# WoodwindHu/RangeLDM

Hardware: AMD Instinct MI355X
Metric: range-images/sec, KITTI-360 64x1024 50-step DDIM @ batch16, 1/2/4/8 GPU (higher is better)
Workload: dtype bf16; 1 GPU; RangeLDM (latent 4x256x16), 50-step DDIM + VAE decode (4x), batch 16 per GPU, synthetic weights, x_T resident in HBM; global_batch=16, batch_per_gpu=16, inference_steps=50, sampler=ddim, parallelism=sample-sharded x1, RCCL all-gather of finished images

## Files before the change

### include/rangeldm_hip.h

```cpp
#ifndef RANGELDM_HIP_H
#define RANGELDM_HIP_H

#include <stddef.h>
#include <stdint.h>

#ifdef __cplusplus
extern "C" {
#endif

#define RLDM_MAX_LEVELS 8

typedef struct rldm_unet rldm_unet;
typedef struct rldm_vae rldm_vae;
typedef struct rldm_sampler rldm_sampler;

typedef struct rldm_unet_config {
    int32_t sample_w, sample_h;
    int32_t in_channels, out_channels;
    int32_t layers_per_block;
    int32_t num_levels;
    int32_t block_out_channels[RLDM_MAX_LEVELS];
    int32_t down_attn[RLDM_MAX_LEVELS];
    int32_t up_attn[RLDM_MAX_LEVELS];
    int32_t attention_head_dim;
// ... 257 lines not shown
    const float* cs1;
    const float* gamma;
    const float* beta;
    int32_t silu, groups;
    float eps;
    float* cs_out;
    const float* g0;
    const float* g1;
    int32_t G0;
    const float* gcs0;
    const float* gcs1;
    const float* ggamma;
    const float* gbeta;
    int32_t gsilu, ggroups;
    float geps;
    float* gs_out;
} rldm_train_fuse;
int rldm_train_conv_fused_ok(const rldm_train_conv_desc* d, const rldm_train_fuse* f, int rowadd_ld);
int rldm_train_conv_fused(const rldm_train_conv_desc* d, const rldm_train_fuse* f, const float* x, const void* w_packed,
                          const float* bias, const float* rowadd, int rowadd_ld, const float* res, float* y, int prezeroed,
                          void* stream);
int rldm_train_wgrad_fused_ok(const rldm_train_conv_desc* d, const rldm_train_fuse* f);
int rldm_train_wgrad_fused(const rldm_train_conv_desc* d, const rldm_train_fuse* f, const float* dy, const float* x, float* dw,
                           float* rows, int rows_ld, int rows_accumulate, float* total, void* stream);
int rldm_train_defer_reduce(int on);
int rldm_train_flush_reduce(void);
int rldm_train_reduce_pending(void);
int rldm_train_wgrad_group(int on);
int rldm_train_wgrad_group_flush(void);
int rldm_train_wgrad_group_pending(void);
int rldm_train_deterministic(int on);
int rldm_train_deterministic_enabled(void);
int rldm_train_chan_stats(const float* x, int B, int npix, int C, float* cs, void* stream);
int rldm_train_gn_backward_apply(const float* dz, const float* x0, const float* x1, int C0, const float* cs0, const float* cs1,
                                 const float* gs, int B, int npix, int C, int groups, float eps, const float* gamma,
                                 const float* res, float* dx0, int accumulate0, float* dx1, int accumulate1, float* dgamma,
                                 float* dbeta, void* stream);
int rldm_train_linear_rows(const float* x, int ldx, const void* w_packed, int K, const float* bias, float* y, int ldy, int B, int N,
                           int accumulate, void* stream);
int rldm_train_linear_rows_wgrad(const float* dy, int ldy, const float* x, int ldx, int B, int N, int K, float* dw, float* dbias,
                                 void* stream);
int rldm_train_attention_forward(const float* q, const float* k, const float* v, int B, int L, int C, float* o, float* lse,
                                 void* stream);
int rldm_train_attention_backward(const float* q, const float* k, const float* v, const float* o, const float* dO, const float* lse,
                                  int B, int L, int C, float* delta, float* dq, float* dk, float* dv, void* stream);
int rldm_train_attention_qkv_forward(const float* qkv, int B, int L, int C, float* o, float* lse, void* stream);
int rldm_train_attention_qkv_backward(const float* qkv, const float* o, const float* dO, const float* lse, int B, int L, int C,
                                      float* delta, float* dqkv, void* stream);
int rldm_train_add(const float* a, const float* b, float* y, int64_t n, void* stream);
int rldm_train_copy_channels(const float* src, int src_ld, int src_off, float* dst, int dst_ld, int dst_off, int ncopy,
                             int64_t npix, int accumulate, void* stream);
int rldm_train_sum2x2(const float* du, int B, int W, int H, int C, float* dx, void* stream);
int rldm_train_silu(const float* x, const float* dy, float* y, int64_t n, int backward, int accumulate, void* stream);
int rldm_train_timestep_embedding(const int64_t* timesteps , int B, int dim, float* out, void* stream);
int rldm_train_pack_input(const float* x, int B, int C, int W, int H, int pos_encoding, float* y, void* stream);
int rldm_train_unpack_output(const float* x, int B, int C, int W, int H, float* y, void* stream);
int rldm_train_mse(const float* pred, const float* target, const float* weight, int B, int C, int W, int H, float* dpred,
                   double* loss, void* stream);
int rldm_train_l1(const float* pred, const float* target, const float* wc, int B, int C, int W, int H, float* dpred, double* out,
                  void* stream);
int rldm_train_gaussian(const float* moments, const float* noise, int B, int W, int H, int Z, float* z, double* kl, void* stream);
int rldm_train_gaussian_backward(const float* moments, const float* noise, const float* dz, float kw, int B, int W, int H, int Z,
                                 float* dmoments, void* stream);
int rldm_train_sqnorm(const float* g, int64_t n, double* out , void* stream);
typedef struct rldm_adamw_config {
    float lr, beta1, beta2, eps, weight_decay;
    float max_grad_norm;
    float ema_decay;
    int32_t step;
} rldm_adamw_config;
int rldm_train_adamw(float* params, const float* grads, float* exp_avg, float* exp_avg_sq, float* ema, const double* sqnorm,
                     int64_t n, const rldm_adamw_config* c, void* stream);
int rldm_train_adamw_dyn(float* params, float* grads, float* exp_avg, float* exp_avg_sq, float* ema, const double* sqnorm,
                         int64_t n, const rldm_adamw_config* c, const float* dyn, int zero_grads, void* stream);
typedef struct rldm_hyper_config {
    float lr, beta1, beta2;
    float ema_max_decay, ema_inv_gamma, ema_power;
    int64_t lr_warmup_steps, total_steps;
} rldm_hyper_config;
int rldm_train_hyper_step(int64_t* step_counter, const rldm_hyper_config* c, float* dyn, void* stream);
int rldm_train_pack_weights(const float* w, int N, int Cin, int taps, void* w_forward, void* w_transposed, void* stream);
typedef struct rldm_pack_desc {
    int64_t first;
    int64_t param_offset;
    void* w_forward;
    void* w_transposed;
    int32_t N, Cin, taps, pad_;
} rldm_pack_desc;
int rldm_train_pack_weights_all(const float* params, const rldm_pack_desc* descs, int num_layers, int64_t total, void* stream);
int rldm_train_pack_weights_tiled(const float* params, const rldm_pack_desc* descs, int num_layers, int64_t total_tiles, void* stream);

typedef struct rldm_train_disc_conv_desc {
    int32_t B, Win, Hin, Cin;
    int32_t N;
    int32_t stride;
} rldm_train_disc_conv_desc;
int rldm_train_disc_conv_ok(const rldm_train_disc_conv_desc* d);
int rldm_train_disc_conv(const rldm_train_disc_conv_desc* d, const float* x, const void* w_packed, const float* bias, float* y,
                         void* stream);
int rldm_train_disc_conv_dgrad(const rldm_train_disc_conv_desc* d, const float* dy, const void* w_transposed, float* dx, void* stream);
int64_t rldm_train_disc_wgrad_workspace(const rldm_train_disc_conv_desc* d);
int rldm_train_disc_wgrad(const rldm_train_disc_conv_desc* d, const float* dy, const float* x, float* dw, float* dbias,
                          void* workspace, int64_t workspace_bytes, void* stream);
int64_t rldm_train_disc_bn_workspace(int64_t M, int C);
int rldm_train_disc_bn_forward(const float* x, int64_t M, int C, const float* gamma, const float* beta, float* running_mean,
                               float* running_var, int64_t* num_batches_tracked, int training, float* save, float* y,
                               void* workspace, int64_t workspace_bytes, void* stream);
int rldm_train_disc_bn_backward(const float* x, const float* dy, const float* save, int64_t M, int C, const float* gamma,
                                const float* beta, float* dx, float* dgamma, float* dbeta, void* workspace, int64_t workspace_bytes,
                                void* stream);
int rldm_train_disc_lrelu(const float* x, const float* dy, float* y, int64_t n, int backward, void* stream);
int rldm_train_disc_hinge(const float* real, const float* fake, int64_t n, float factor, float* dreal, float* dfake, double* out,
                          double* partials, void* stream);
int rldm_train_disc_generator(const float* fake, int64_t n, float* dfake, double* out, double* partials, void* stream);
int rldm_train_disc_adaptive_mix(const float* dnll, const float* dg, const double* sq_nll, const double* sq_g, float disc_weight,
                                 float disc_factor, float* dpred, double* d_weight, int64_t n, void* stream);

typedef struct rldm_train_meta_desc {
    int32_t B, Win, Hin, C;
    int32_t N;
    int32_t stride;
} rldm_train_meta_desc;
int rldm_train_meta_ok(const rldm_train_meta_desc* d);
int64_t rldm_train_meta_workspace(const rldm_train_meta_desc* d);
int rldm_train_meta_range(const float* x, int64_t npix, int C, float range_mean, float range_std, float* r, void* stream);
int rldm_train_meta_range_grad(const float* dr, int64_t npix, int C, float range_std, float* dx, void* stream);
int rldm_train_meta_forward(const rldm_train_meta_desc* d, const float* x, const float* r, const float* tables, const float* w1,
                            const float* b1, const float* w2, const float* b2, const float* coov, const float* bias, float* y,
                            float* r_next, float* pe, int32_t* src, float* m, void* workspace, int64_t workspace_bytes, void* stream);
int rldm_train_meta_backward(const rldm_train_meta_desc* d, const float* x, const float* dy, const float* tables, const float* w1,
                             const float* b1, const float* w2, const float* coov, const float* pe, const int32_t* src, const float* m,
                             const float* dr_next, float* dx, float* dr, float* dw1, float* db1, float* dw2, float* db2, float* dcoov,
                             float* dbias, void* workspace, int64_t workspace_bytes, void* stream);

double rldm_unet_flops(rldm_unet* m, int B);
double rldm_vae_decode_flops(rldm_vae* m, int B, int latent_w, int latent_h);
int rldm_unet_num_launches(rldm_unet* m, int B);

int rldm_sampler_profile(rldm_sampler* s, const float* x_T, char* json_out, size_t cap);

typedef struct rldm_conv_desc {
    int32_t B, Cin0, Cin1, Win, Hin;
    int32_t Cout;
    int32_t ksize;
    int32_t stride;
    int32_t pad_mode;
    int32_t upsample;
    int32_t gn;
    int32_t silu;
    float eps;
} rldm_conv_desc;
int rldm_test_conv(const rldm_conv_desc* d, const float* x0, const float* x1, const float* weight, const float* bias,
                   const float* gamma, const float* beta, const float* temb, const float* res, float* y, void* stream);
int rldm_bench_conv(const rldm_conv_desc* d, int with_res, int with_temb, int warmup, int iters, float* avg_us,
                    char* kernel_name, size_t name_cap, void* stream);
int rldm_debug_force_tile(int BM, int BN, int ksplit);
int rldm_unet_trunk_status(rldm_unet* m, int B);
int rldm_unet_set_plan_flags(rldm_unet* m, int flags);
int rldm_debug_inject_trunk_error(rldm_sampler* s, int code);
int rldm_debug_timestamps(unsigned long long* host_out);
int rldm_debug_block_times(unsigned long long* host_out, int nblocks);
enum rldm_flag {
    RLDM_FLAG_ATTN_PROJ_LAUNCH = 1 << 7,
    RLDM_FLAG_NO_CONV_SMALL    = 1 << 8,
    RLDM_FLAG_SMALL_128PX      = 1 << 10,
    RLDM_FLAG_NO_STREAM_REGW   = 1 << 11,
    RLDM_FLAG_STREAM_ANY_GRID  = 1 << 12,
    RLDM_FLAG_GRAPH_TRACE      = 1 << 13,
    RLDM_FLAG_SMALL_64PX_32X2  = 1 << 19,
    RLDM_FLAG_CONSUMER_GN      = 1 << 20,
    RLDM_FLAG_NO_WIDE_SPLIT    = 1 << 21,
    RLDM_FLAG_OWN_IMAGE_COPIES = 1 << 22,
    RLDM_FLAG_SCHED_LAUNCH     = 1 << 23,
    RLDM_FLAG_NO_PERSISTENT    = 1 << 24,
    RLDM_FLAG_NO_CLUSTERS      = 1 << 26
};
int rldm_debug_set_flags(int flags);
enum rldm_flag2 {
    RLDM_FLAG2_STREAM_8WAVE_FULL = 1,
    RLDM_FLAG2_STREAM_8WAVE_128X8 = 2,
    RLDM_FLAG2_STREAM_8WAVE_C64 = 4,
    RLDM_FLAG2_STREAM_SPEC_WAVES = 32,
    RLDM_FLAG2_STREAM_64PX = 64,
    RLDM_FLAG2_NO_REGW = 1 << 24,
    RLDM_FLAG2_REGW_CAP8 = 1 << 25,
    RLDM_FLAG2_FP32_OUT = 1 << 26,
    RLDM_FLAG2_HALO_RING = 1 << 29
};
int rldm_debug_set_flags2(int flags);
int rldm_debug_graph_trace(unsigned long long* stamps, int cap, char* names, size_t names_cap);
int rldm_test_conv_stats(const rldm_conv_desc* d, const float* x0, const float* weight, const float* bias, float* stats,
                         void* stream);
int rldm_test_attention(const float* qkv, int B, int L, int C, float* out, void* stream);
int rldm_test_attention_qkv(const float* x, int B, int L, int C, int groups, float eps, const float* gamma, const float* beta,
                            const float* wqkv, const float* bqkv, float* out, void* stream);
int rldm_test_attention_route(int B, int L, int C, int* route);
int rldm_test_attention_block(const float* x, int B, int L, int C, int groups, float eps, const float* gamma, const float* beta,
                              const float* wqkv, const float* bqkv, const float* to_out_w, const float* to_out_b, int mode, float* y,
                              float* stats, void* stream);
int rldm_bench_attention_qkv(int B, int L, int C, int warmup, int iters, float* avg_us, void* stream);

int rldm_calibrate(double* mfma_tflops, double* mfma_clock_mhz, double* copy_gbs, void* stream);
#define RLDM_CALIB_STAMP_BLOCKS 16
int rldm_calib_clock_stamp(unsigned long long* slots, void* stream);

#ifdef __cplusplus
}
#endif
#endif
```

### rangeldm_amd/_lib.py

```python
import ctypes as C
import enum
import os

_HERE = os.path.dirname(os.path.abspath(__file__))
LIB_PATH = os.environ.get("RLDM_LIB") or os.path.join(_HERE, "librangeldm_hip.so")
RLDM_MAX_LEVELS = 8
RLDM_SAMPLER_DDIM, RLDM_SAMPLER_DDPM, RLDM_SAMPLER_DPMSOLVER = 0, 1, 2
RLDM_EMD_RECT, RLDM_EMD_SYMMETRIC, RLDM_EMD_DIAGONAL = 0, 1, 2
RLDM_EMD_BID_CAP = 2
RLDM_VOXEL_RANGE, RLDM_VOXEL_MAX_SLOTS = 4, 1 << 25
RLDM_HOUGH_MAX_THETA, RLDM_HOUGH_MAX_H, RLDM_HOUGH_MAX_BEAMS = 65536, 4096, 256
RLDM_FRECHET_SWEEP_CAP, RLDM_FRECHET_NONFINITE, RLDM_FRECHET_MAX_SWEEPS = 2, 3, 60
RLDM_FEATURE_MAX_K = 16
RLDM_TRAIN_PAD_END = 4
RLDM_RN_CONV1X1, RLDM_RN_CONV3X3, RLDM_RN_CONV3X3_S2, RLDM_RN_UPCONV = 0, 1, 2, 3


class Flag(enum.IntFlag):
    ATTN_PROJ_LAUNCH = 1 << 7
    NO_CONV_SMALL = 1 << 8
    SMALL_128PX = 1 << 10
    NO_STREAM_REGW = 1 << 11
    STREAM_ANY_GRID = 1 << 12
    GRAPH_TRACE = 1 << 13
    SMALL_64PX_32X2 = 1 << 19
    CONSUMER_GN = 1 << 20
    NO_WIDE_SPLIT = 1 << 21
    OWN_IMAGE_COPIES = 1 << 22
    SCHED_LAUNCH = 1 << 23
    NO_PERSISTENT = 1 << 24
    NO_CLUSTERS = 1 << 26


class Flag2(enum.IntFlag):
    STREAM_8WAVE_FULL = 1
    STREAM_8WAVE_128X8 = 2
    STREAM_8WAVE_C64 = 4
    STREAM_SPEC_WAVES = 32
    STREAM_64PX = 64
    NO_REGW = 1 << 24
    REGW_CAP8 = 1 << 25
    FP32_OUT = 1 << 26
    HALO_RING = 1 << 29


class UNetConfigC(C.Structure):
    _fields_ = [("sample_w", C.c_int32), ("sample_h", C.c_int32), ("in_channels", C.c_int32),
                ("out_channels", C.c_int32), ("layers_per_block", C.c_int32), ("num_levels", C.c_int32),
                ("block_out_channels", C.c_int32 * RLDM_MAX_LEVELS), ("down_attn", C.c_int32 * RLDM_MAX_LEVELS),
                ("up_attn", C.c_int32 * RLDM_MAX_LEVELS), ("attention_head_dim", C.c_int32),
                ("norm_num_groups", C.c_int32), ("norm_eps", C.c_float), ("mid_attention", C.c_int32),
                ("flip_sin_to_cos", C.c_int32), ("freq_shift", C.c_int32)]


class VAEConfigC(C.Structure):
    _fields_ = [("in_channels", C.c_int32), ("out_channels", C.c_int32), ("ch", C.c_int32), ("num_levels", C.c_int32),
                ("ch_mult", C.c_int32 * RLDM_MAX_LEVELS), ("num_res_blocks", C.c_int32), ("z_channels", C.c_int32),
                ("double_z", C.c_int32), ("norm_num_groups", C.c_int32), ("norm_eps", C.c_float),
                ("scaling_factor", C.c_float)]


class SamplerConfigC(C.Structure):
    _fields_ = [("batch", C.c_int32), ("num_steps", C.c_int32), ("mode", C.c_int32), ("pos_encoding", C.c_int32),
                ("cond_channels", C.c_int32), ("guided", C.c_int32), ("coef", C.POINTER(C.c_float)),
                ("timesteps", C.POINTER(C.c_int64)),
                ("plan_flags", C.c_int32), ("prediction_type", C.c_int32)]


class ConvDescC(C.Structure):
    _fields_ = [("B", C.c_int32), ("Cin0", C.c_int32), ("Cin1", C.c_int32), ("Win", C.c_int32), ("Hin", C.c_int32),
                ("Cout", C.c_int32), ("ksize", C.c_int32), ("stride", C.c_int32), ("pad_mode", C.c_int32),
                ("upsample", C.c_int32), ("gn", C.c_int32), ("silu", C.c_int32), ("eps", C.c_float)]


class LidarConfigC(C.Structure):
    _fields_ = [("beams", C.c_int32), ("width", C.c_int32), ("mode", C.c_int32), ("mean", C.c_float), ("std", C.c_float),
                ("range_fill", C.c_float), ("intensity_fill", C.c_float), ("grid", C.c_int32 * 3),
                ("pc_range", C.c_float * 6), ("normalize_volume_densities", C.c_int32)]


class RangeNetLayerDescC(C.Structure):
    _fields_ = [("kind", C.c_int32), ("B", C.c_int32), ("H", C.c_int32), ("W", C.c_int32), ("Cin", C.c_int32),
                ("Cout", C.c_int32), ("leaky", C.c_int32)]


class RangeNetConfigC(C.Structure):
    _fields_ = [("layers", C.c_int32), ("in_channels", C.c_int32), ("num_classes", C.c_int32)]


class TrainConvDescC(C.Structure):
    _fields_ = [("B", C.c_int32), ("Win", C.c_int32), ("Hin", C.c_int32), ("Cin", C.c_int32), ("N", C.c_int32),
                ("taps", C.c_int32), ("stride", C.c_int32), ("mode", C.c_int32)]


class TrainMetaDescC(C.Structure):
    _fields_ = [("B", C.c_int32), ("Win", C.c_int32), ("Hin", C.c_int32), ("C", C.c_int32), ("N", C.c_int32), ("stride", C.c_int32)]


class TrainDiscConvDescC(C.Structure):
    _fields_ = [("B", C.c_int32), ("Win", C.c_int32), ("Hin", C.c_int32), ("Cin", C.c_int32), ("N", C.c_int32), ("stride", C.c_int32)]


class TrainFuseC(C.Structure):
    _fields_ = [("x1", C.c_void_p), ("C0", C.c_int32), ("cs0", C.c_void_p), ("cs1", C.c_void_p), ("gamma", C.c_void_p),
                ("beta", C.c_void_p), ("silu", C.c_int32), ("groups", C.c_int32), ("eps", C.c_float), ("cs_out", C.c_void_p),
                ("g0", C.c_void_p), ("g1", C.c_void_p), ("G0", C.c_int32), ("gcs0", C.c_void_p), ("gcs1", C.c_void_p),
                ("ggamma", C.c_void_p), ("gbeta", C.c_void_p), ("gsilu", C.c_int32), ("ggroups", C.c_int32), ("geps", C.c_float),
                ("gs_out", C.c_void_p)]


class PackDescC(C.Structure):
    _fields_ = [("first", C.c_int64), ("param_offset", C.c_int64), ("w_forward", C.c_void_p), ("w_transposed", C.c_void_p),
                ("N", C.c_int32), ("Cin", C.c_int32), ("taps", C.c_int32), ("pad_", C.c_int32)]


class HyperConfigC(C.Structure):
    _fields_ = [("lr", C.c_float), ("beta1", C.c_float), ("beta2", C.c_float), ("ema_max_decay", C.c_float),
                ("ema_inv_gamma", C.c_float), ("ema_power", C.c_float), ("lr_warmup_steps", C.c_int64), ("total_steps", C.c_int64)]


class AdamWConfigC(C.Structure):
    _fields_ = [("lr", C.c_float), ("beta1", C.c_float), ("beta2", C.c_float), ("eps", C.c_float),
                ("weight_decay", C.c_float), ("max_grad_norm", C.c_float), ("ema_decay", C.c_float), ("step", C.c_int32)]


_P = C.c_void_p
PROTOTYPES = {
    "rldm_last_error": (C.c_char_p, []),
    "rldm_device_info": (C.c_int, [C.c_char_p, C.c_size_t, C.POINTER(C.c_int)]),
    "rldm_unet_create": (C.c_int, [C.POINTER(UNetConfigC), C.POINTER(_P)]),
    "rldm_unet_destroy": (None, [_P]),
    "rldm_unet_set_param": (C.c_int, [_P, C.c_char_p, _P, C.c_int64]),
    "rldm_unet_finalize": (C.c_int, [_P]),
    "rldm_unet_forward": (C.c_int, [_P, _P, _P, C.c_int, C.c_int, _P, _P]),
    "rldm_vae_create": (C.c_int, [C.POINTER(VAEConfigC), C.POINTER(_P)]),
    "rldm_vae_destroy": (None, [_P]),
    "rldm_vae_set_param": (C.c_int, [_P, C.c_char_p, _P, C.c_int64]),
    "rldm_vae_finalize": (C.c_int, [_P]),
    "rldm_vae_decode": (C.c_int, [_P, _P, C.c_int, C.c_int, C.c_int, _P, _P]),
    "rldm_vae_encode": (C.c_int, [_P, _P, C.c_int, C.c_int, C.c_int, _P, _P]),
    "rldm_diag_gaussian_sample": (C.c_int, [_P, _P, C.c_float, C.c_int, C.c_int, C.c_int, _P, _P]),
    "rldm_sched_ddim_step": (C.c_int, [C.POINTER(C.c_float), _P, _P, _P, _P, C.c_int64, _P]),
    "rldm_sched_ddpm_step": (C.c_int, [C.POINTER(C.c_float), _P, _P, _P, _P, C.c_int64, _P]),
    "rldm_sched_step": (C.c_int, [C.c_int, C.c_int, C.POINTER(C.c_float), _P, _P, _P, _P, C.c_int64, _P]),
    "rldm_sched_dpmsolver_step": (C.c_int, [C.c_int, C.POINTER(C.c_float), _P, _P, _P, _P, C.c_int64, _P]),
    "rldm_sched_guided_step": (C.c_int, [C.c_int, C.c_int, C.POINTER(C.c_float), _P, _P, _P, _P, _P, _P, _P, _P, C.c_int, C.c_int,
                                         C.c_int64, _P]),
    "rldm_sched_add_noise": (C.c_int, [_P, _P, C.POINTER(C.c_float), C.POINTER(C.c_float), C.c_int, C.c_int64, _P, _P]),
    "rldm_sampler_create": (C.c_int, [_P, _P, C.POINTER(SamplerConfigC), C.POINTER(_P)]),
    "rldm_sampler_destroy": (None, [_P]),
    "rldm_sample": (C.c_int, [_P, _P, _P, _P, _P, _P, _P]),
    "rldm_sample_guided": (C.c_int, [_P, _P, _P, _P, _P, _P, _P, _P, _P, _P]),
    "rldm_sampler_status": (C.c_int, [_P]),
    "rldm_unet_set_plan_flags": (C.c_int, [_P, C.c_int]),
    "rldm_debug_inject_trunk_error": (C.c_int, [_P, C.c_int]),
    "rldm_comm_bind": (C.c_int, []),
    "rldm_comm_unique_id": (C.c_int, [_P, C.c_size_t]),
    "rldm_comm_create": (C.c_int, [_P, C.c_int, C.c_int, C.POINTER(_P)]),
    "rldm_comm_destroy": (None, [_P]),
    "rldm_comm_info": (C.c_int, [_P, C.POINTER(C.c_int), C.POINTER(C.c_int), C.c_char_p, C.c_size_t]),
    "rldm_allgather_images": (C.c_int, [_P, _P, _P, C.c_int64, _P]),
    "rldm_allreduce_grads": (C.c_int, [_P, _P, C.c_int64, C.c_int, _P]),
    "rldm_lidar_create": (C.c_int, [C.POINTER(LidarConfigC), C.POINTER(C.c_float), C.POINTER(C.c_float), C.POINTER(_P)]),
    "rldm_lidar_destroy": (None, [_P]),
    "rldm_lidar_to_points": (C.c_int, [_P, _P, C.c_int, C.c_int, C.c_int, _P, _P]),
    "rldm_lidar_to_voxel": (C.c_int, [_P, _P, C.c_int, C.c_int, C.c_int, _P, _P]),
    "rldm_lidar_to_voxel_train": (C.c_int, [_P, _P, C.c_int, C.c_int, C.c_int, _P, _P, _P]),
    "rldm_lidar_to_voxel_ordered": (C.c_int, [_P, _P, C.c_int, C.c_int, C.c_int, _P, _P, _P]),
    "rldm_lidar_to_voxel_backward": (C.c_int, [_P, _P, C.c_int, C.c_int, C.c_int, _P, _P, _P, _P, _P]),
    "rldm_lidar_filter_points": (C.c_int, [_P, _P, C.c_int, C.c_int, C.c_int, C.c_float, _P, _P, _P]),
    "rldm_render_u8": (C.c_int, [_P, C.c_int, C.c_int, C.c_int, C.c_int, C.c_int, _P, _P]),
    "rldm_lidar_project": (C.c_int, [_P, _P, C.c_int, C.c_int, _P, C.c_float, _P, _P, _P, _P]),
    "rldm_bev_histogram": (C.c_int, [_P, _P, C.c_int, C.c_int, C.c_float, C.c_int, C.c_float, C.c_float, _P, _P]),
    "rldm_hist_jsd": (C.c_int, [_P, C.c_int, _P, C.c_int, C.c_int, C.POINTER(C.c_double), _P]),
    "rldm_hist_spectral_sq": (C.c_int, [_P, C.c_int, _P, C.c_int, C.c_int, C.c_int, _P, _P]),
    "rldm_hist_mmd": (C.c_int, [_P, C.c_int, _P, C.c_int, C.c_int, C.c_float, C.POINTER(C.c_double), _P]),
    "rldm_chamfer_nn": (C.c_int, [_P, _P, C.c_int, _P, _P, C.c_int, C.c_int, _P, _P, _P]),
    "rldm_chamfer_mean": (C.c_int, [_P, _P, _P, _P, C.c_int, _P, _P, _P]),
    "rldm_nn_index": (C.c_int, [_P, _P, C.c_int, _P, _P, C.c_int, C.c_int, _P, _P, _P, _P, _P, _P, _P]),
    "rldm_knn": (C.c_int, [_P, _P, C.c_int, _P, _P, C.c_int, C.c_int, C.c_int, C.c_int, _P, _P, _P]),
    "rldm_knn_normals": (C.c_int, [_P, _P, C.c_int, C.c_int, _P, C.c_int, _P, _P, _P]),
    "rldm_chamfer_matrix": (C.c_int, [_P, _P, C.c_int, C.c_int, _P, _P, C.c_int, C.c_int, C.c_int, _P, _P, _P]),
    "rldm_matrix_row_argmin": (C.c_int, [_P, C.c_int, C.c_int, C.c_int, _P, _P, _P]),
    "rldm_voxel_counts": (C.c_int, [_P, _P, C.c_int, _P, _P, C.c_int, C.c_int, C.c_float, _P, _P]),
    "rldm_hough_pack": (C.c_int, [_P, C.c_int64, C.c_int, C.c_float, C.c_float, _P, _P]),
    "rldm_hough_vote": (C.c_int, [_P, C.c_int64, _P, C.c_int, C.c_float, C.c_float, C.c_int, _P, _P]),
    "rldm_hough_vote_shape": (C.c_int, [C.c_int64, C.c_int, C.c_int, C.POINTER(C.c_int32), C.POINTER(C.c_int64)]),
    "rldm_hough_row_max": (C.c_int, [_P, C.c_int, C.c_int, _P, _P, _P]),
    "rldm_hough_assign": (C.c_int, [_P, C.c_int64, _P, C.c_int, C.c_float, _P, _P]),
    "rldm_hough_moments": (C.c_int, [_P, _P, C.c_int64, C.c_int, _P, _P, _P]),
    "rldm_emd_matrix": (C.c_int, [_P, _P, C.c_int, C.c_int, _P, _P, C.c_int, C.c_int, C.c_int, C.c_float, _P, _P, _P, _P, _P]),
    "rldm_farthest_point_sample": (C.c_int, [_P, _P, C.c_int, C.c_int, C.c_int, _P, _P, _P]),
    "rldm_gram_f64": (C.c_int, [_P, C.c_int, _P, C.c_int, C.c_int, _P, _P]),
    "rldm_singular_values_f64": (C.c_int, [_P, C.c_int, C.c_int, C.c_double, C.c_int, _P, C.POINTER(C.c_int), _P]),
    "rldm_frechet_distance": (C.c_int, [_P, C.c_int, _P, C.c_int, C.c_int, C.POINTER(C.c_double), _P]),
    "rldm_frechet_last_sweeps": (C.c_int, []),
    "rldm_feature_scan_f64": (C.c_int, [_P, C.c_int, _P, C.c_int, C.c_int, C.c_int, _P, _P, C.c_int, C.c_int, C.c_longlong,
                                        _P, _P, _P, _P, _P, _P]),
    "rldm_feature_scan_column_chunk": (C.c_int, [C.c_int]),
    "rldm_rangenet_packed_elems": (C.c_longlong, [C.c_int, C.c_int, C.c_int]),
    "rldm_rangenet_pack_weights": (C.c_int, [C.c_int, C.c_int, C.c_int, _P, _P]),
    "rldm_rangenet_layer": (C.c_int, [C.POINTER(RangeNetLayerDescC), _P, _P, _P, _P, _P, _P, _P, _P, _P, _P, C.c_int, _P, _P, _P]),
    "rldm_rangenet_num_layers": (C.c_int, [C.POINTER(RangeNetConfigC)]),
    "rldm_rangenet_layer_info": (C.c_int, [C.POINTER(RangeNetConfigC), C.c_int, C.POINTER(RangeNetLayerDescC)]),
    "rldm_rangenet_create": (C.c_int, [C.POINTER(RangeNetConfigC), C.POINTER(_P), C.POINTER(_P), C.POINTER(_P), C.c_int, C.POINTER(_P)]),
    "rldm_rangenet_destroy": (None, [_P]),
    "rldm_rangenet_forward": (C.c_int, [_P, _P, C.c_int, C.c_int, C.c_int, _P, _P, C.c_int, _P, _P, _P, _P]),
    "rldm_rangenet_project": (C.c_int, [_P, _P, C.c_int, C.c_int, C.c_int, C.c_int, C.c_double, C.c_double, C.POINTER(C.c_float),
                                        C.POINTER(C.c_float), _P, _P, _P, _P, _P, _P, _P, _P, _P]),
    "rldm_rangenet_unproject": (C.c_int, [_P, _P, _P, _P, _P, _P, C.c_int, C.c_int, C.c_int, C.c_int, C.c_int, _P, C.c_float,
                                          C.c_int, _P, _P]),
    "rldm_range_errors": (C.c_int, [_P, _P, C.c_int, C.c_int, C.c_int, C.c_int, C.c_int, C.POINTER(C.c_float),
                                    C.POINTER(C.c_float), C.c_int, C.c_int, _P, _P, _P]),
    "rldm_beam_upsample": (C.c_int, [_P, C.c_int, C.c_int, C.c_int, C.c_int, C.c_int, C.c_int, _P, _P]),
    "rldm_train_conv": (C.c_int, [C.POINTER(TrainConvDescC), _P, _P, _P, _P, C.c_int, _P, _P, C.c_int, _P]),
    "rldm_train_conv_splits": (C.c_int, [C.POINTER(TrainConvDescC), C.c_int]),
    "rldm_train_wgrad": (C.c_int, [C.POINTER(TrainConvDescC), _P, _P, _P, _P]),
    "rldm_train_wgrad_bias": (C.c_int, [C.POINTER(TrainConvDescC), _P, _P, _P, _P, C.c_int, C.c_int, _P, _P]),
    "rldm_train_colsum": (C.c_int, [_P, C.c_int, C.c_int, C.c_int, _P, C.c_int, C.c_int, _P, _P]),
    "rldm_train_gn_forward": (C.c_int, [_P, C.c_int, C.c_int, C.c_int, C.c_int, C.c_float, _P, _P, C.c_int, _P, _P, _P]),
    "rldm_train_gn_backward": (C.c_int, [_P, _P, _P, C.c_int, C.c_int, C.c_int, C.c_int, _P, _P, C.c_int, _P, _P, C.c_int,
                                         _P, _P, _P]),
    "rldm_train_conv_fused_ok": (C.c_int, [C.POINTER(TrainConvDescC), C.POINTER(TrainFuseC), C.c_int]),
    "rldm_train_conv_fused": (C.c_int, [C.POINTER(TrainConvDescC), C.POINTER(TrainFuseC), _P, _P, _P, _P, C.c_int, _P, _P, C.c_int, _P]),
    "rldm_train_wgrad_fused_ok": (C.c_int, [C.POINTER(TrainConvDescC), C.POINTER(TrainFuseC)]),
    "rldm_train_wgrad_fused": (C.c_int, [C.POINTER(TrainConvDescC), C.POINTER(TrainFuseC), _P, _P, _P, _P, C.c_int, C.c_int, _P, _P]),
    "rldm_train_defer_reduce": (C.c_int, [C.c_int]),
    "rldm_train_flush_reduce": (C.c_int, []),
    "rldm_calibrate": (C.c_int, [C.POINTER(C.c_double), C.POINTER(C.c_double), C.POINTER(C.c_double), _P]),
    "rldm_calib_clock_stamp": (C.c_int, [_P, _P]),
    "rldm_train_wgrad_group": (C.c_int, [C.c_int]),
    "rldm_train_wgrad_group_flush": (C.c_int, []),
    "rldm_train_wgrad_group_pending": (C.c_int, []),
    "rldm_train_deterministic": (C.c_int, [C.c_int]),
    "rldm_train_deterministic_enabled": (C.c_int, []),
    "rldm_train_reduce_pending": (C.c_int, []),
    "rldm_train_chan_stats": (C.c_int, [_P, C.c_int, C.c_int, C.c_int, _P, _P]),
    "rldm_train_gn_backward_apply": (C.c_int, [_P, _P, _P, C.c_int, _P, _P, _P, C.c_int, C.c_int, C.c_int, C.c_int, C.c_float, _P, _P,
                                               _P, C.c_int, _P, C.c_int, _P, _P, _P]),
    "rldm_train_linear_rows": (C.c_int, [_P, C.c_int, _P, C.c_int, _P, _P, C.c_int, C.c_int, C.c_int, C.c_int, _P]),
    "rldm_train_linear_rows_wgrad": (C.c_int, [_P, C.c_int, _P, C.c_int, C.c_int, C.c_int, C.c_int, _P, _P, _P]),
    "rldm_train_attention_forward": (C.c_int, [_P, _P, _P, C.c_int, C.c_int, C.c_int, _P, _P, _P]),
    "rldm_train_attention_backward": (C.c_int, [_P, _P, _P, _P, _P, _P, C.c_int, C.c_int, C.c_int, _P, _P, _P, _P, _P]),
    "rldm_train_attention_qkv_forward": (C.c_int, [_P, C.c_int, C.c_int, C.c_int, _P, _P, _P]),
    "rldm_train_attention_qkv_backward": (C.c_int, [_P, _P, _P, _P, C.c_int, C.c_int, C.c_int, _P, _P, _P]),
    "rldm_train_add": (C.c_int, [_P, _P, _P, C.c_int64, _P]),
    "rldm_train_copy_channels": (C.c_int, [_P, C.c_int, C.c_int, _P, C.c_int, C.c_int, C.c_int, C.c_int64, C.c_int, _P]),
    "rldm_train_sum2x2": (C.c_int, [_P, C.c_int, C.c_int, C.c_int, C.c_int, _P, _P]),
    "rldm_train_silu": (C.c_int, [_P, _P, _P, C.c_int64, C.c_int, C.c_int, _P]),
    "rldm_train_timestep_embedding": (C.c_int, [_P, C.c_int, C.c_int, _P, _P]),
    "rldm_train_pack_input": (C.c_int, [_P, C.c_int, C.c_int, C.c_int, C.c_int, C.c_int, _P, _P]),
    "rldm_train_unpack_output": (C.c_int, [_P, C.c_int, C.c_int, C.c_int, C.c_int, _P, _P]),
    "rldm_train_mse": (C.c_int, [_P, _P, _P, C.c_int, C.c_int, C.c_int, C.c_int, _P, _P, _P]),
    "rldm_train_l1": (C.c_int, [_P, _P, _P, C.c_int, C.c_int, C.c_int, C.c_int, _P, _P, _P]),
    "rldm_train_gaussian": (C.c_int, [_P, _P, C.c_int, C.c_int, C.c_int, C.c_int, _P, _P, _P]),
    "rldm_train_gaussian_backward": (C.c_int, [_P, _P, _P, C.c_float, C.c_int, C.c_int, C.c_int, C.c_int, _P, _P]),
    "rldm_train_sqnorm": (C.c_int, [_P, C.c_int64, _P, _P]),
    "rldm_train_adamw": (C.c_int, [_P, _P, _P, _P, _P, _P, C.c_int64, C.POINTER(AdamWConfigC), _P]),
    "rldm_train_adamw_dyn": (C.c_int, [_P, _P, _P, _P, _P, _P, C.c_int64, C.POINTER(AdamWConfigC), _P, C.c_int, _P]),
    "rldm_train_hyper_step": (C.c_int, [_P, C.POINTER(HyperConfigC), _P, _P]),
    "rldm_train_pack_weights": (C.c_int, [_P, C.c_int, C.c_int, C.c_int, _P, _P, _P]),
    "rldm_train_pack_weights_all": (C.c_int, [_P, _P, C.c_int, C.c_int64, _P]),
    "rldm_train_pack_weights_tiled": (C.c_int, [_P, _P, C.c_int, C.c_int64, _P]),
    "rldm_train_disc_conv_ok": (C.c_int, [C.POINTER(TrainDiscConvDescC)]),
    "rldm_train_disc_conv": (C.c_int, [C.POINTER(TrainDiscConvDescC), _P, _P, _P, _P, _P]),
    "rldm_train_disc_conv_dgrad": (C.c_int, [C.POINTER(TrainDiscConvDescC), _P, _P, _P, _P]),
    "rldm_train_disc_wgrad_workspace": (C.c_int64, [C.POINTER(TrainDiscConvDescC)]),
    "rldm_train_disc_wgrad": (C.c_int, [C.POINTER(TrainDiscConvDescC), _P, _P, _P, _P, _P, C.c_int64, _P]),
    "rldm_train_disc_bn_workspace": (C.c_int64, [C.c_int64, C.c_int]),
    "rldm_train_disc_bn_forward": (C.c_int, [_P, C.c_int64, C.c_int, _P, _P, _P, _P, _P, C.c_int, _P, _P, _P, C.c_int64, _P]),
    "rldm_train_disc_bn_backward": (C.c_int, [_P, _P, _P, C.c_int64, C.c_int, _P, _P, _P, _P, _P, _P, C.c_int64, _P]),
    "rldm_train_disc_lrelu": (C.c_int, [_P, _P, _P, C.c_int64, C.c_int, _P]),
    "rldm_train_disc_hinge": (C.c_int, [_P, _P, C.c_int64, C.c_float, _P, _P, _P, _P, _P]),
    "rldm_train_disc_generator": (C.c_int, [_P, C.c_int64, _P, _P, _P, _P]),
    "rldm_train_disc_adaptive_mix": (C.c_int, [_P, _P, _P, _P, C.c_float, C.c_float, _P, _P, C.c_int64, _P]),
    "rldm_train_meta_ok": (C.c_int, [C.POINTER(TrainMetaDescC)]),
    "rldm_train_meta_workspace": (C.c_int64, [C.POINTER(TrainMetaDescC)]),
    "rldm_train_meta_range": (C.c_int, [_P, C.c_int64, C.c_int, C.c_float, C.c_float, _P, _P]),
    "rldm_train_meta_range_grad": (C.c_int, [_P, C.c_int64, C.c_int, C.c_float, _P, _P]),
    "rldm_train_meta_forward": (C.c_int, [C.POINTER(TrainMetaDescC)] + [_P] * 15 + [C.c_int64, _P]),
    "rldm_train_meta_backward": (C.c_int, [C.POINTER(TrainMetaDescC)] + [_P] * 20 + [C.c_int64, _P]),
    "rldm_unet_flops": (C.c_double, [_P, C.c_int]),
    "rldm_vae_decode_flops": (C.c_double, [_P, C.c_int, C.c_int, C.c_int]),
    "rldm_unet_num_launches": (C.c_int, [_P, C.c_int]),
    "rldm_unet_trunk_status": (C.c_int, [_P, C.c_int]),
    "rldm_sampler_profile": (C.c_int, [_P, _P, C.c_char_p, C.c_size_t]),
    "rldm_test_conv": (C.c_int, [C.POINTER(ConvDescC), _P, _P, _P, _P, _P, _P, _P, _P, _P, _P]),
    "rldm_bench_conv": (C.c_int, [C.POINTER(ConvDescC), C.c_int, C.c_int, C.c_int, C.c_int, C.POINTER(C.c_float),
                                  C.c_char_p, C.c_size_t, _P]),
    "rldm_debug_force_tile": (C.c_int, [C.c_int, C.c_int, C.c_int]),
    "rldm_test_conv_stats": (C.c_int, [C.POINTER(ConvDescC), _P, _P, _P, _P, _P]),
    "rldm_debug_set_flags": (C.c_int, [C.c_int]),
    "rldm_debug_set_flags2": (C.c_int, [C.c_int]),
    "rldm_debug_graph_trace": (C.c_int, [_P, C.c_int, C.c_char_p, C.c_size_t]),
    "rldm_debug_timestamps": (C.c_int, [_P]),
    "rldm_debug_block_times": (C.c_int, [_P, C.c_int]),
    "rldm_test_attention": (C.c_int, [_P, C.c_int, C.c_int, C.c_int, _P, _P]),
    "rldm_test_attention_qkv": (C.c_int, [_P, C.c_int, C.c_int, C.c_int, C.c_int, C.c_float, _P, _P, _P, _P, _P, _P]),
    "rldm_test_attention_route": (C.c_int, [C.c_int, C.c_int, C.c_int, C.POINTER(C.c_int)]),
    "rldm_test_attention_block": (C.c_int, [_P, C.c_int, C.c_int, C.c_int, C.c_int, C.c_float, _P, _P, _P, _P, _P, _P, C.c_int, _P, _P,
                                            _P]),
    "rldm_bench_attention_qkv": (C.c_int, [C.c_int, C.c_int, C.c_int, C.c_int, C.c_int, C.POINTER(C.c_float), _P]),
}

_lib = None


def lib():
    global _lib
    if _lib is None:
        if not os.path.exists(LIB_PATH):
            raise RuntimeError(f"{LIB_PATH} not found: build it with `python -c 'import __graft_entry__ as g; g.build()'` "
                               f"(hipcc --offload-arch=gfx950).  rangeldm_amd has no CPU fallback.")
        import torch
        L = C.CDLL(LIB_PATH)
        for name, (res, args) in PROTOTYPES.items():
            fn = getattr(L, name)
            fn.restype = res
            fn.argtypes = args
        _lib = L
    return _lib


def check(rc, what=""):
    if rc != 0:
        msg = lib().rldm_last_error()
        raise RuntimeError(f"librangeldm_hip: {what} failed: {msg.decode() if msg else 'unknown error'}")


def stream_ptr(device=None):
    import torch
    return C.c_void_p(torch.cuda.current_stream(device).cuda_stream)


def require_gpu():
    import torch
    if not torch.cuda.is_available():
        raise RuntimeError("rangeldm_amd needs an MI355X (gfx950) visible to PyTorch-ROCm; there is no CPU fallback")
    name = C.create_string_buffer(64)
    cus = C.c_int(0)
    check(lib().rldm_device_info(name, 64, C.byref(cus)), "rldm_device_info")
    return name.value.decode(), cus.value
```

### rangeldm_amd/csrc/conv_stream.hip

```cpp
#include "conv_stream_body.h"
#include "conv_stream_spec_body.h"

#include <utility>

namespace rldm {

template <int WM, int WN, int NW, int MI, int S, bool SUB, bool T4, bool FH>
__global__ void __launch_bounds__((StreamInstDesc{WM, WN, NW, MI}.threads()), (StreamInstDesc{WM, WN, NW, MI}.wg_per_cu())) conv_stream_kernel(const ConvParams p) {
    int nt, mt, b;
    {
        const int gx = p.ntile_n, gy = p.tiles_img;
        const int lin = blockIdx.x + gx * (blockIdx.y + gy * blockIdx.z);
        const int rid = (p.dbg & (1 << 21)) ? lin : xcd_remap(lin, gx * gy * p.B);
        const int q = rid / gx;
        nt = rid - q * gx;
        b = q / gy;
        mt = q - b * gy;
    }
    const TrunkSeam none = {};
    conv_stream_body<WM, WN, false, NW, MI, S, SUB, T4, FH>(p, nt, mt, b, none);
}

__global__ void __launch_bounds__(512, 1) conv_stream_spec_kernel(const ConvParams p) {
    int nt, mt, b;
    {
        const int gx = p.ntile_n, gy = p.tiles_img;
        const int lin = blockIdx.x + gx * (blockIdx.y + gy * blockIdx.z);
        const int rid = (p.dbg & (1 << 21)) ? lin : xcd_remap(lin, gx * gy * p.B);
        const int q = rid / gx;
        nt = rid - q * gx;
        b = q / gy;
        mt = q - b * gy;
    }
    const TrunkSeam none = {};
    conv_stream_spec_body<false>(p, nt, mt, b, none);
}

int conv_stream_bn(const ConvParams& p) { return stream_inst(p).bn(); }
int conv_stream_kgroups(const ConvParams& p) { return stream_inst(p).kgroups(); }
int conv_stream_threads(const ConvParams& p) { return stream_inst(p).threads(); }

size_t conv_stream_lds_bytes(const ConvParams& p) {
    const int BN = conv_stream_bn(p), KG = conv_stream_kgroups(p), BM = p.TW * p.TH;
    const size_t a = (size_t)((p.TW - 1) * p.stride + 3) * p.colb;
    const size_t main_bytes = 2 * a + (size_t)(p.C0 + p.C1) * 8 + BN * 4;
    const size_t gscratch = p.st0 ? (size_t)2 * (p.C0 + p.C1) * 8 : 0;
    const size_t epi = KG == 1 ? (size_t)BM * (BN * 2 + 16) + (size_t)8 * 2 * BN * 4
                               : (size_t)KG * 64 * (BN * 4 + 16) + (size_t)64 * (BN * 2 + 16) + (size_t)8 * 2 * BN * 4;
    return std::max(std::max(main_bytes, gscratch), epi);
}

bool conv_stream_supported(const ConvParams& p, int taps) {
    if (p.st_inst < 0 || p.st_inst >= SI_COUNT) return false;
    const StreamInstDesc& d = stream_inst(p);
    const int Cin = p.C0 + p.C1, R = p.R0 + p.R1;
    if (taps != 9 || p.pad_lo != 1 || (p.up != 1 && p.up != 2) || p.y_nchw || p.ksplit > 1) return false;
    if (Cin % 64 != 0 || (p.C1 != 0 && p.C0 % 64 != 0) || R % 64 != 0 || (p.R1 != 0 && p.R0 % 64 != 0)) return false;
    if (R != 0 && p.up != 1) return false;
    if (p.Win * p.up < 2 || p.N % d.bn() != 0 || Cin > 512) return false;
    if (p.st0 && (p.gn_groups > 64 || Cin % p.gn_groups != 0)) return false;
    if ((p.tiles_h & (p.tiles_h - 1)) != 0 || p.B > 65535 || p.tiles_img > 65535) return false;
    if (p.stride != d.STR || !d.takes(p.TW, p.TH) || (d.up1 && p.up != 1) || (d.no_res && R != 0)) return false;
    if (d.SUB && (p.Wout != 2 * p.Win || p.Hout != 2 * p.Hin)) return false;
    if (d.FH && p.Hout != p.TH) return false;
    return conv_stream_lds_bytes(p) <= (size_t)d.lds_cap();
}

template <int I>
static int launch_stream_inst(const ConvParams& p, size_t lds, hipStream_t stream) {
    constexpr StreamInstDesc d = kStreamInst[I];
    void (*kern)(const ConvParams);
    if constexpr (d.spec) kern = conv_stream_spec_kernel;
    else kern = conv_stream_kernel<d.WM, d.WN, d.NW, d.MI, d.STR, d.SUB, d.T4, d.FH>;
    static DynLdsLimit lds_limit;
    RLDM_HIP_CHECK(lds_limit.ensure(reinterpret_cast<const void*>(kern), lds));
    hipLaunchKernelGGL(kern, dim3(p.N / d.bn() * (d.SUB ? 4 : 1), p.tiles_img, p.B), dim3(d.threads()), lds, stream, p);
    RLDM_HIP_CHECK(hipGetLastError());
    return 0;
}
template <int... I>
static int launch_stream_row(const ConvParams& p, size_t lds, hipStream_t stream, std::integer_sequence<int, I...>) {
    static constexpr int (*launch[])(const ConvParams&, size_t, hipStream_t) = {launch_stream_inst<I>...};
    return launch[p.st_inst](p, lds, stream);
}

int launch_conv_stream(const ConvParams& p, hipStream_t stream) {
    RLDM_REQUIRE(conv_stream_supported(p, 9), "conv_stream: unsupported shape");
    return launch_stream_row(p, conv_stream_lds_bytes(p), stream, std::make_integer_sequence<int, SI_COUNT>());
}

}
```

### rangeldm_amd/csrc/kernels.h

```cpp
#pragma once
#include "common.h"

namespace rldm {

struct NormView {
    bf16_t* y;
    const float* gamma;
    const float* beta;
    int ld;
    int cpg_shift;
    float inv_n;
    float eps;
    int silu;
};

constexpr int kSchedMultistep = 8;
__device__ __forceinline__ float sched_prev(const int mode, const float c0, const float c1, const float c2, const float c3, const float x,
                                            const float e, float& x0_out) {
    const int pred = (mode >> 1) & 3;
    float x0, pe;
    if (pred == 0) {
        x0 = (x - c1 * e) / c0;
        pe = e;
    } else if (pred == 1) {
        x0 = c0 * x - c1 * e;
        pe = c0 * e + c1 * x;
    } else {
        x0 = e;
        pe = (x - c0 * e) / c1;
    }
    x0_out = x0;
    return (mode & 1) == 0 ? c2 * x0 + c3 * pe : c2 * x0 + c3 * x;
}
__device__ __forceinline__ float* sched_history(const int mode, const float* slot) {
    return (mode & kSchedMultistep) ? const_cast<float*>(slot) : nullptr;
}

struct SchedFuse {
    const float* coef_table;
    const int* step_ptr;
    const float* x;
    const float* noise;
    long long noise_step_stride;
    float* x_prev;
    int mode;
    bf16_t* pack;
    int pack_ld;
};

struct ConvParams {
    const bf16_t* x0;
    const bf16_t* x1;
    int C0, C1;
    const bf16_t* r0;
    const bf16_t* r1;
    int R0, R1;
    int B, Win, Hin;
    int up;
    int stride;
    int pad_lo;
    int Wout, Hout;
    int TW, TH;
    int colb;
    int tiles_h, tiles_img;
    int th_shift;
    int magic_thv;
    int magic_cpg;
    const float2* st0;
    const float2* st1;
    int P0, P1;
    int gn_groups;
    const float* gn_gamma;
    const float* gn_beta;
    float gn_eps;
    int silu;
    const bf16_t* wpk;
    int N;
    int ntile_n;
    const float* bias;
    const float* temb;
    int temb_ld;
    const int* step_ptr;
    int temb_rows_per_step;
    int temb_per_sample;
    bf16_t* y;
    int y_ld;
    float2* y_stats;
    float* y_nchw;
    int ksplit;
    float* slab;
    int* ticket;
    int lds_total;
    float gn_inv_n;
    const bf16_t* res;
    unsigned long long* ts;
    int dbg;
    SchedFuse sch;
    int* step_inc;
    int nviews;
    NormView nv[3];
    int st_inst;
    int exp;
    int* cu_lock;
};

struct ConvTile {
    int BM, BN, CK, taps;
};
inline int conv_row_bytes(int CK) { return CK * 2 + 16; }
size_t conv_lds_bytes(const ConvTile& t, const ConvParams& p);
bool conv_tile_supported(const ConvTile& t);
int conv_max_halo_slots(const ConvTile& t);
int conv_halo_col_bytes(const ConvTile& t, int TH, int stride);
int conv_tile_threads(const ConvTile& t);
int launch_conv(const ConvTile& t, const ConvParams& p, hipStream_t stream);

int conv_small_kgroups(int BN);
int conv_small_col_bytes(int Cin, int TH, int taps);
size_t conv_small_lds_bytes(const ConvParams& p, int taps, int BN);
bool conv_small_supported(const ConvParams& p, int taps, int BN);
int launch_conv_small(const ConvParams& p, int taps, int BN, hipStream_t stream);

enum StreamInst : int {
    SI_256x128,
    SI_256x64,
    SI_128x64,
    SI_256x128_SPEC,
    SI_64x128,
    SI_64x128_S2,
    SI_128x128_W4,
    SI_128x64_W4,
    SI_SUB_W4,
    SI_SUB_T4_W4,
    SI_FULLH_W4,
    SI_COUNT
};
enum TrunkStreamForm : int { TSF_NONE = -1, TSF_PLAIN = 0, TSF_SUB = 1, TSF_FULLH = 2 };
struct StreamTile {
    int TW, TH;
};
struct StreamInstDesc {
    int WM, WN, NW = 8, MI = 4, STR = 1;
    bool SUB = false, T4 = false, FH = false;
    bool spec = false;
    StreamTile tiles[2] = {};
    bool up1 = false, no_res = false;
    int trunk = TSF_NONE;
    constexpr int threads() const { return 64 * NW; }
    constexpr int kgroups() const { return NW / (WM * WN); }
    constexpr int bm() const { return 32 * MI * WM; }
    constexpr int bn() const { return 32 * WN; }
    constexpr int wg_per_cu() const { return NW == 4 ? 2 : 1; }
    constexpr int lds_cap() const { return 160 * 1024 / wg_per_cu(); }
    constexpr bool takes(int TW, int TH) const { return (tiles[0].TW == TW && tiles[0].TH == TH) || (tiles[1].TW == TW && tiles[1].TH == TH); }
};
constexpr StreamInstDesc kStreamInst[SI_COUNT] = {
     {2, 4, 8, 4, 1, false, false, false, false, {{32, 8}},          false, false, TSF_PLAIN},
     {2, 2, 8, 4, 1, false, false, false, false, {{32, 8}}},
     {1, 2, 8, 4, 1, false, false, false, false, {{16, 8}, {32, 4}}},
     {2, 4, 8, 4, 1, false, false, false, true,  {{32, 8}}},
     {1, 4, 8, 2, 1, false, false, false, false, {{8, 8}}},
     {1, 4, 8, 2, 2, false, false, false, false, {{8, 8}, {16, 4}},  true,  true},
     {1, 4, 4, 4, 1, false, false, false, false, {{16, 8}},          false, false, TSF_PLAIN},
     {1, 2, 4, 4, 1, false, false, false, false, {{16, 8}}},
     {1, 4, 4, 4, 1, true,  false, false, false, {{16, 8}},          true,  true,  TSF_SUB},
     {1, 4, 4, 4, 1, true,  true,  false, false, {{32, 4}},          true,  true},
     {1, 4, 4, 4, 1, false, false, true,  false, {{8, 16}, {16, 8}}, true,  false, TSF_FULLH},
};
inline const StreamInstDesc& stream_inst(const ConvParams& p) { return kStreamInst[p.st_inst]; }
int conv_stream_bn(const ConvParams& p);
int conv_stream_kgroups(const ConvParams& p);
size_t conv_stream_lds_bytes(const ConvParams& p);
bool conv_stream_supported(const ConvParams& p, int taps);
int launch_conv_stream(const ConvParams& p, hipStream_t stream);

size_t conv_regw_lds_bytes();
int conv_regw_wg_per_image(const ConvParams& p);
int conv_regw_partials(const ConvParams& p);
bool conv_regw_supported(const ConvParams& p);
int launch_conv_regw(const ConvParams& p, hipStream_t stream);
size_t conv_c16_lds_bytes();
bool conv_c16_supported(const ConvParams& p);
int launch_conv_c16(const ConvParams& p, hipStream_t stream);
size_t conv_o4_lds_bytes();
bool conv_o4_supported(const ConvParams& p);
int launch_conv_o4(const ConvParams& p, hipStream_t stream);
size_t conv_ds2_lds_bytes();
bool conv_ds2_supported(const ConvParams& p);
int launch_conv_ds2(const ConvParams& p, hipStream_t stream);

struct TrunkPhase;
struct TrunkParams {
    const TrunkPhase* phases;
    int nphases;
    int B, ranks;
    int ntile_n, nwn;
    int variant;
    int skew;
    unsigned* counters;
    int* error;
    const float* temb;
    const int* step_ptr;
    int temb_rows_per_step, temb_per_sample, temb_ld;
    unsigned long long* ts;
};
int launch_trunk(const TrunkParams& tp, size_t lds, hipStream_t stream);
int trunk_max_resident(int variant, size_t lds);

struct GnStatsParams {
    const bf16_t* x;
    int C;
    int B, npix;
    int P;
    float2* part;
};
int launch_gn_stats(const GnStatsParams& p, hipStream_t stream);

struct GnFoldParams {
    const float2* part;
    float2* out;
    int B, P, C;
};
int launch_gn_fold(const GnFoldParams& p, hipStream_t stream);

struct GnApplyParams {
    const bf16_t* x0;
    const bf16_t* x1;
    int C0, C1;
    const float2* st0;
    const float2* st1;
    int P0, P1;
    int B, npix;
    int groups;
    const float* gamma;
    const float* beta;
    float eps;
    int silu;
    bf16_t* y;
    float inv_n;
    bf16_t* y1;
    int ysplit;
};
int launch_gn_apply(const GnApplyParams& p, hipStream_t stream);

struct AttnParams {
    const bf16_t* qkv;
    bf16_t* out;
    int B, L, C;
};
int launch_attention(const AttnParams& p, hipStream_t stream);

struct AttnQkvParams {
    const bf16_t* x;
    const float2* st;
    int P;
    const float* gamma;
    const float* beta;
    float eps;
    int groups;
    float inv_n;
    int magic_cpg;
    const bf16_t* wfrag;
    const float* bias;
    bf16_t* out;
    int B, L, C;
    unsigned long long* ts;
    int ts_L;
    const bf16_t* proj_w;
    const float* proj_bias;
    const bf16_t* proj_res;
    bf16_t* proj_y;
    float2* proj_stats;
    unsigned* proj_counter;
    int* proj_error;
};
int launch_attention_qkv(const AttnQkvParams& p, hipStream_t stream);
int attention_qkv2_geometry(int B, int L, int C, int* HG, int* waves);
bool attention_proj_fusable(int B, int L, int C, int cus);
int launch_attention_proj(const AttnQkvParams& p, hipStream_t stream);
void attention_qkv_route(int B, int L, int C, int cus, int* route);
constexpr int kAttnXRowBytes = 128 + 16, kAttnXStageBytes = 32 * kAttnXRowBytes;
inline size_t attention_qkv2_lds_bytes(int L, int C, int HG, int waves) {
    const size_t Lp = (size_t)(L + 31) / 32 * 32;
    const size_t a = (size_t)2 * C * 8, b2 = (size_t)HG * (C / 16) * 64 * 4;
    return HG * Lp * 16 + (size_t)HG * 10 * (Lp + 8) * 2 + 16 + (size_t)C * 8 + (a > b2 ? a : b2) + (size_t)HG * C * 64 +
           (size_t)HG * 128 + (size_t)waves * kAttnXStageBytes + 128;
}

struct PackInputParams {
    const float* x; int cx; float scale;
    int pos_encoding;
    const float* cond; int cc;
    int B, W, H, Cpad;
    bf16_t* out;
    int* step_inc;
};
int launch_pack_input(const PackInputParams& p, hipStream_t stream);
int launch_nchw_f32_to_nhwc_bf16(const float* src, bf16_t* dst, int B, int C, int W, int H, int Cpad, hipStream_t s);
int launch_nhwc_bf16_to_nchw_f32(const bf16_t* src, float* dst, int B, int C, int W, int H, int ld, hipStream_t s);

struct TembParams {
    const float* t;
    int rows, dim0, D, total;
    const float* w1; const float* b1;
    const float* w2; const float* b2;
    const float* wp; const float* bp;
    float* out;
    float* scratch;
    int flip_sin_to_cos, freq_shift;
};
int launch_temb(const TembParams& p, hipStream_t stream);

struct SchedParams {
    int mode;
    float coef[5];
    const float* coef_table;
    const int* step_ptr;
    const float* eps; const float* x; const float* noise;
    long long noise_step_stride;
    float* x_prev;
    long long n;
};
int launch_sched_step(const SchedParams& p, hipStream_t stream);
struct GuidedSchedParams {
    SchedParams s;
    float k[4];
// ... 19 lines not shown
```

### rangeldm_amd/csrc/runtime.hip

```cpp
#include "../../include/rangeldm_hip.h"
#include "kernels.h"
#include "trunk_seam.h"

#include <algorithm>
#include <atomic>
#include <cmath>
#include <cstdlib>
#include <cstring>
#include <functional>
#include <map>
#include <memory>
#include <mutex>
#include <tuple>
#include <vector>

namespace rldm {

static thread_local std::string g_error;
void set_error(const std::string& msg) { g_error = msg; }

struct DevBuf {
    void* p = nullptr;
    size_t bytes = 0;
    DevBuf() = default;
// ... 127 lines not shown
            RLDM_REQUIRE(ksize == 3 && (Cout % 32 == 0 || Cout < 32) && Cin_pad % 64 == 0 && R % 64 == 0, "conv " + name + ": not stream-packable");
            const int SPT = 4 / KG, NCC = Cin_pad / 64, NCB = R / 64, nsteps = (NCC * 9 + NCB) * SPT;
            const int ntile32 = (Cout + 31) / 32;
            img.assign((size_t)ntile32 * KG * nsteps * 512 + 16384, 0);
            auto at = [&](int n, int ks, int step, int k) -> bf16_t& {
                const size_t stream = (size_t)(n / 32) * KG + ks / SPT;
                return img[((stream * nsteps + step + ks % SPT) * 64 + (k / 8) * 32 + n % 32) * 8 + k % 8];
            };
            for (int n = 0; n < Cout; ++n) {
                for (int c = 0; c < Cin; ++c)
                    for (int tap = 0; tap < 9; ++tap) at(n, (c % 64) / 16, ((c / 64) * 9 + tap) * SPT, c % 16) = f32_to_bf16(weight(n, c, tap));
                for (int c = 0; c < R; ++c) at(n, (c % 64) / 16, (NCC * 9 + c / 64) * SPT, c % 16) = f32_to_bf16(res_weight(n, c));
            }
            bias.resize((size_t)ntile32 * 32, 0.f);
            return 0;
        });
    }

    int get_c16packed(Packed** out) {
        return cached({WeightLayout::C16, 0, 0}, 16, out, [&](std::vector<bf16_t>& img, std::vector<float>&) {
            RLDM_REQUIRE(ksize == 3 && Cout % 32 == 0 && Cin <= 16 && R == 0, "conv " + name + ": not a 16-channel input layer");
            img.assign((size_t)(Cout / 32) * 9 * 512, 0);
            for (int n = 0; n < Cout; ++n)
                for (int c = 0; c < Cin; ++c)
                    for (int tap = 0; tap < 9; ++tap)
                        img[(((size_t)(n / 32) * 9 + tap) * 64 + (c / 8) * 32 + n % 32) * 8 + c % 8] = f32_to_bf16(weight(n, c, tap));
            return 0;
        });
    }

    int get_subpixpacked(int Cin_pad, Packed** out) {
        return cached({WeightLayout::SubPixel, 0, 0}, Cin_pad, out, [&](std::vector<bf16_t>& img, std::vector<float>&) {
            RLDM_REQUIRE(ksize == 3 && Cout % 32 == 0 && Cin_pad % 64 == 0 && R == 0, "conv " + name + ": not sub-pixel-packable");
            const int NCC = Cin_pad / 64, nsteps = NCC * 16;
            img.assign((size_t)(Cout / 32) * 4 * nsteps * 512 + 16384, 0);
            static const int lo[2][2] = {{0, 1}, {0, 2}}, hi[2][2] = {{0, 2}, {1, 2}};
            for (int n = 0; n < Cout; ++n)
                for (int c = 0; c < Cin; ++c)
                    for (int pw = 0; pw < 2; ++pw)
                        for (int ph = 0; ph < 2; ++ph)
                            for (int i = 0; i < 2; ++i)
                                for (int j = 0; j < 2; ++j) {
                                    float v = 0.f;
                                    for (int a = lo[pw][i]; a <= hi[pw][i]; ++a)
                                        for (int bb = lo[ph][j]; bb <= hi[ph][j]; ++bb) v += weight(n, c, a * 3 + bb);
                                    const size_t stream = (size_t)(n / 32) * 4 + pw * 2 + ph;
                                    const int step = ((c / 64) * 4 + i * 2 + j) * 4 + (c % 64) / 16, k = c % 16;
                                    img[((stream * nsteps + step) * 64 + (k / 8) * 32 + n % 32) * 8 + k % 8] = f32_to_bf16(v);
                                }
            return 0;
        });
    }

    int get_fragpacked(int Cin_pad, int TN, int KG, bool no_res, Packed** out) {
        const WeightLayout layout = no_res ? WeightLayout::FragNoRes : WeightLayout::Frag;
        return cached({layout, TN, KG}, Cin_pad, out, [&](std::vector<bf16_t>& img, std::vector<float>&) {
            const int taps = ksize * ksize, Rp = no_res ? 0 : R, KS = 512 / TN;
            RLDM_REQUIRE((TN == 32 || TN == 16) && Cout % TN == 0 && Cin_pad % (KS * KG) == 0 && Rp % (KS * KG) == 0,
                         "conv " + name + ": not fragment-packable");
            const int CPT = Cin_pad / KS / KG, RPT = Rp / KS / KG, nmine = taps * CPT + RPT;
            img.assign((size_t)(Cout / TN) * KG * nmine * 512 + 512, 0);
            auto at = [&](int n, int step0, int c) -> bf16_t& {
                const int cg = c / KS, k = c % KS;
                const size_t stream = (size_t)(n / TN) * KG + cg % KG;
                return img[((stream * nmine + step0 + cg / KG) * 64 + (k / 8) * TN + n % TN) * 8 + k % 8];
            };
            for (int n = 0; n < Cout; ++n) {
                for (int c = 0; c < Cin; ++c)
                    for (int tap = 0; tap < taps; ++tap) at(n, tap * CPT, c) = f32_to_bf16(weight(n, c, tap));
                for (int c = 0; c < Rp; ++c) at(n, taps * CPT, c) = f32_to_bf16(res_weight(n, c));
            }
            return 0;
        });
    }
};

struct ParamStore {
    std::map<std::string, std::vector<float>> host;
    std::map<std::string, int64_t> expected;
    bool finalized = false;

    int set(const char* name, const float* data, int64_t numel) {
        auto it = expected.find(name);
        RLDM_REQUIRE(it != expected.end(), std::string("unexpected parameter key: ") + name);
        RLDM_REQUIRE(it->second == numel, std::string("size mismatch for ") + name + ": expected " +
                                              std::to_string(it->second) + " got " + std::to_string(numel));
        host[name].assign(data, data + numel);
        finalized = false;
        return 0;
    }
    int check_complete() const {
        for (auto& kv : expected)
            RLDM_REQUIRE(host.count(kv.first), std::string("missing parameter key: ") + kv.first);
        return 0;
    }
    void expect_conv(const std::string& n, int co, int ci, int k) {
        expected[n + ".weight"] = (int64_t)co * ci * k * k;
        expected[n + ".bias"] = co;
    }
    void expect_lin(const std::string& n, int co, int ci) {
        expected[n + ".weight"] = (int64_t)co * ci;
        expected[n + ".bias"] = co;
    }
    void expect_norm(const std::string& n, int c) {
        expected[n + ".weight"] = c;
        expected[n + ".bias"] = c;
    }
    void expect_resnet(const std::string& p, int ci, int co, int temb) {
        expect_norm(p + ".norm1", ci);
        expect_conv(p + ".conv1", co, ci, 3);
        if (temb) expect_lin(p + ".time_emb_proj", co, temb);
        expect_norm(p + ".norm2", co);
        expect_conv(p + ".conv2", co, co, 3);
        if (ci != co) expect_conv(p + ".conv_shortcut", co, ci, 1);
    }
    void expect_attn(const std::string& p, int c) {
        expect_norm(p + ".group_norm", c);
        expect_lin(p + ".to_q", c, c);
        expect_lin(p + ".to_k", c, c);
        expect_lin(p + ".to_v", c, c);
        expect_lin(p + ".to_out.0", c, c);
    }
};

struct Tensor {
    size_t off = 0;
    int B = 0, W = 0, H = 0, C = 0;
    int id = -1;
    size_t st_off = 0;
    int P = 0;
    int prod = -1;
    size_t st_bytes() const { return (size_t)B * P * C * sizeof(float2); }
    size_t bytes() const { return (size_t)B * W * H * C * sizeof(bf16_t); }
    bool valid() const { return id >= 0; }
};

struct PlanIO {
    const float* sample = nullptr;
    int sample_channels = 0;
    float sample_scale = 1.f;
    int pos_encoding = 0;
    const float* cond = nullptr;
    int cond_channels = 0;
    float* out = nullptr;
    const float* temb = nullptr;
    const int* step_ptr = nullptr;
    int temb_rows_per_step = 1;
    int temb_per_sample = 0;
    int* step_inc = nullptr;
    SchedFuse sch = {};
    bool pack_fused = false;
    bf16_t* xin = nullptr;
    int xin_ld = 0;
};

struct Op {
    std::function<int(hipStream_t)> fn;
    std::string name;
    double flops = 0;
    double bytes = 0;
    std::function<bool()> active;
    std::string tag;
};

struct KernelStat {
    int launches = 0;
    double ms = 0, flops = 0, bytes = 0;
};

struct Plan {
    int B = 0, W = 0, H = 0;
    int flags = 0;
    DevBuf arena;
    DevBuf tickets;
    std::vector<std::unique_ptr<DevBuf>> trunk_bufs;
    DevBuf trunk_error;
    PlanIO io;
    std::vector<Op> ops;
    double flops = 0;
    int run(hipStream_t s) {
        for (auto& o : ops)
            if ((!o.active || o.active()) && o.fn(s)) return 1;
        return 0;
    }
    int run_stamped(hipStream_t s, unsigned long long* slots, int cap) {
        if (launch_stamp(slots, s)) return 1;
        int n = 0;
        for (size_t i = 0; i < ops.size(); ++i) {
            if (ops[i].active && !ops[i].active()) continue;
            if (ops[i].fn(s)) return 1;
            ++n;
            if (n < cap && launch_stamp(slots + n, s)) return 1;
        }
        return 0;
    }
    int run_profiled(hipStream_t s, std::map<std::string, KernelStat>& stats) {
        std::vector<hipEvent_t> ev(ops.size() + 1);
        for (auto& e : ev) RLDM_HIP_CHECK(hipEventCreate(&e));
        RLDM_HIP_CHECK(hipEventRecord(ev[0], s));
        std::vector<char> ran(ops.size(), 1);
        for (size_t i = 0; i < ops.size(); ++i) {
            ran[i] = !ops[i].active || ops[i].active();
            if (ran[i] && ops[i].fn(s)) return 1;
            RLDM_HIP_CHECK(hipEventRecord(ev[i + 1], s));
        }
        RLDM_HIP_CHECK(hipStreamSynchronize(s));
        for (size_t i = 0; i < ops.size(); ++i) {
            if (!ran[i]) continue;
            float ms = 0.f;
            RLDM_HIP_CHECK(hipEventElapsedTime(&ms, ev[i], ev[i + 1]));
            KernelStat& k = stats[ops[i].name];
            k.launches += 1;
            k.ms += ms;
            k.flops += ops[i].flops;
            k.bytes += ops[i].bytes;
        }
        for (auto& e : ev) (void)hipEventDestroy(e);
        return 0;
    }
};

struct Layers {
    std::map<std::string, std::unique_ptr<ConvLayer>> conv;
    std::map<std::string, std::unique_ptr<NormParams>> norm;
    ConvLayer* get_conv(const std::string& n) {
        auto it = conv.find(n);
        return it == conv.end() ? nullptr : it->second.get();
    }
    NormParams* get_norm(const std::string& n) {
        auto it = norm.find(n);
        return it == norm.end() ? nullptr : it->second.get();
    }
    int add_conv(ParamStore& ps, const std::string& n, int co, int ci, int k) {
        auto L = std::make_unique<ConvLayer>();
        L->name = n;
        L->Cout = co;
        L->Cin = ci;
        L->ksize = k;
        L->w = ps.host.at(n + ".weight");
        L->b = ps.host.at(n + ".bias");
        conv[n] = std::move(L);
        return 0;
    }
    int add_norm(ParamStore& ps, const std::string& n, int c) {
        auto N = std::make_unique<NormParams>();
        N->C = c;
        if (upload(N->gamma, ps.host.at(n + ".weight").data(), c * sizeof(float))) return 1;
        if (upload(N->beta, ps.host.at(n + ".bias").data(), c * sizeof(float))) return 1;
        norm[n] = std::move(N);
        return 0;
    }
    int add_qkv(ParamStore& ps, const std::string& p, int c, int head_dim) {
        auto L = std::make_unique<ConvLayer>();
        L->name = p + ".qkv";
        L->Cout = 3 * c;
        L->Cin = c;
        L->ksize = 1;
        const float qs = 1.4426950408889634f / std::sqrt((float)head_dim);
        const char* names[3] = {".to_q", ".to_k", ".to_v"};
        for (int i = 0; i < 3; ++i) {
            const auto& w = ps.host.at(p + names[i] + ".weight");
            const auto& b = ps.host.at(p + names[i] + ".bias");
            const float s = i == 0 ? qs : 1.f;
            for (float v : w) L->w.push_back(v * s);
            for (float v : b) L->b.push_back(v * s);
        }
        conv[L->name] = std::move(L);
        return 0;
    }
};

static void pack_attn_head_frags(const float* w, const float* b, int C, std::vector<bf16_t>& img, std::vector<float>& bias) {
    const int heads = C / 8, nks = C / 16;
    img.assign((size_t)heads * nks * 512, 0);
    bias.assign((size_t)heads * 32, 0.f);
    for (int h = 0; h < heads; ++h)
        for (int row = 0; row < 24; ++row) {
            const int src = (row / 8) * C + h * 8 + row % 8;
            bias[(size_t)h * 32 + row] = b[src];
            for (int c = 0; c < C; ++c)
                img[(((size_t)h * nks + c / 16) * 64 + ((c % 16) / 8) * 32 + row) * 8 + c % 8] = f32_to_bf16(w[(size_t)src * C + c]);
        }
}

struct ConvArgs {
    ConvLayer* layer = nullptr;
    Tensor x0, x1;
    int stride = 1, pad_mode = 0, up = 1;
    NormParams* gn = nullptr;
    float eps = 1e-5f;
    int groups = 32;
    int silu = 0;
    int temb_off = -1;
    Tensor r0, r1;
    bool want_stats = false;
    bool out_f32_nchw = false;
    bool own_image = false;
    bool first_of_step = false;
};

struct ConvShape {
    int Cin_t, R_t, taps, Wout, Hout;
};
static ConvShape conv_shape(const ConvArgs& a) {
    return {a.x0.C + (a.x1.valid() ? a.x1.C : 0), (a.r0.valid() ? a.r0.C : 0) + (a.r1.valid() ? a.r1.C : 0),
            a.layer->ksize * a.layer->ksize, a.x0.W * a.up / a.stride, a.x0.H * a.up / a.stride};
}
static double conv_flops(const ConvArgs& a, const ConvShape& s) {
    const ConvLayer* L = a.layer;
    return 2.0 * (double)a.x0.B * s.Wout * s.Hout * L->Cout * ((double)L->Cin * s.taps + (L->sc_identity ? 0.0 : (double)L->R));
}
static double conv_bytes(const ConvArgs& a, const ConvShape& s, size_t out_copies = 1, bool res_weights = true) {
    const ConvLayer* L = a.layer;
    const double out_px = (double)a.x0.B * s.Wout * s.Hout;
    return (double)a.x0.B * a.x0.W * a.x0.H * s.Cin_t * 2.0 + (double)L->Cout * (L->Cin * s.taps + (res_weights ? L->R : 0)) * 2.0 +
           out_px * L->Cout * (a.out_f32_nchw ? 4.0 : 2.0) * (double)out_copies + out_px * s.R_t * 2.0;
}

struct ConvLate {
    int temb_off = -1;
    bool first_of_step = false;
    bool f32_out = false;
    bool sch = false;
    void apply(ConvParams& p, const PlanIO& io) const {
        if (first_of_step) p.step_inc = io.pack_fused ? io.step_inc : nullptr;
        if (temb_off >= 0) {
            p.temb = io.temb + temb_off;
            p.step_ptr = io.step_ptr;
            p.temb_rows_per_step = io.temb_rows_per_step;
            p.temb_per_sample = io.temb_per_sample;
        }
        if (f32_out) p.y_nchw = io.out;
        if (sch) p.sch = io.sch;
    }
};

struct ViewPlan {
    struct Part { int prod; int ch_off; };
    struct Cons {
        std::vector<Part> parts;
        int Ctot = 0, silu = 0, groups = 32;
        float eps = 1e-5f;
        bool ok = false;
        bool use = false;
    };
    struct Emit { const NormParams* norm; int ch_off; int Ctot; int silu; int groups; float eps; };
    std::vector<char> can_emit;
    std::vector<int> out_c;
    std::map<const NormParams*, Cons> cons;
    std::map<int, std::vector<Emit>> emit;
    void decide() {
        std::map<int, int> nper;
        for (auto& kv : cons) {
            Cons& c = kv.second;
            bool good = c.ok && c.groups > 0 && c.Ctot % c.groups == 0;
            const int cpg = good ? c.Ctot / c.groups : 0;
            good = good && cpg >= 1 && cpg <= 32 && (cpg & (cpg - 1)) == 0;
            for (auto& pt : c.parts)
                good = good && pt.prod >= 0 && pt.prod < (int)can_emit.size() && can_emit[pt.prod] && pt.ch_off % cpg == 0 &&
                       nper[pt.prod] < 3;
            c.use = good;
            if (!good) continue;
            for (auto& pt : c.parts) {
                emit[pt.prod].push_back({kv.first, pt.ch_off, c.Ctot, c.silu, c.groups, c.eps});
                nper[pt.prod]++;
            }
        }
    }
};

static int g_dbg_flags = getenv("RLDM_DBG_FLAGS") ? atoi(getenv("RLDM_DBG_FLAGS")) : 0;
static thread_local int t_plan_flags = 0;
static inline int dbg() { return g_dbg_flags | t_plan_flags; }
static int g_dbg_flags2 = 0;
static inline int dbg2() { return g_dbg_flags2; }
static inline int kernel_dbg() {
#ifdef RLDM_ABLATE
    return dbg();
#else
    return 0;
#endif
}
static unsigned long long* g_ts_buf = nullptr;
struct StampEnv {
    const char *trunk, *trunk_first, *attn_l, *ord;
};
static const StampEnv& stamp_env() {
    static const StampEnv e = {getenv("RLDM_TS_TRUNK"), getenv("RLDM_TS_TRUNK_FIRST"), getenv("RLDM_TS_ATTN_L"), getenv("RLDM_TS_ORD")};
    return e;
}
enum class StampSite { Conv, Attn, TestAttn, Trunk };
static unsigned long long* stamp_buf(StampSite site, int n = 0) {
    const StampEnv& e = stamp_env();
    switch (site) {
        case StampSite::Conv:     return e.ord ? (atoi(e.ord) == n ? g_ts_buf : nullptr) : (e.attn_l || e.trunk) ? nullptr : g_ts_buf;
        case StampSite::Attn:     return (e.trunk || e.ord) ? nullptr : g_ts_buf;
        case StampSite::TestAttn: return e.trunk ? nullptr : g_ts_buf;
        case StampSite::Trunk:    return (e.trunk && atoi(e.trunk) == n) ? g_ts_buf : nullptr;
    }
    return nullptr;
}
static constexpr int kInst4MinBlocks = 96;
static int g_force_bm = 0, g_force_bn = 0, g_force_ks = 0;
static constexpr int kGraphSteps = 10;

static thread_local int g_concurrent_plans = 1;

struct TileChoice {
    ConvTile tile;
    int TW = 1, TH = 1, ksplit = 1;
};

static void pixel_tile(int BM, int Wout, int Hout, int* TW, int* TH) {
    int th = 1;
    while (th * 2 <= Hout && th * 2 <= 16 && Hout % (th * 2) == 0) th *= 2;
    int tw = 1;
    while (tw * 2 * th <= BM && Wout % (tw * 2) == 0) tw *= 2;
    *TW = tw;
    *TH = th;
}

static TileChoice choose_tile(long long B, int Wout, int Hout, int stride, int N, int Cin_pad, int C0, int R, int R0,
                              int taps, bool nchw, bool gn) {
    TileChoice c;
    const int KW = taps == 9 ? 3 : 1;
    auto ck_ok = [&](int ck) { return Cin_pad % ck == 0 && C0 % ck == 0 && R % ck == 0 && R0 % ck == 0; };
    auto pick = [&](int BM, int BN, ConvTile* u, int* tw, int* th) {
        const int cks[3] = {64, 32, 16};
        for (int ck : cks) {
            if (!ck_ok(ck)) continue;
            ConvTile v;
            v.BM = BM; v.BN = BN; v.CK = ck; v.taps = taps;
            if (!conv_tile_supported(v)) continue;
            pixel_tile(BM, Wout, Hout, tw, th);
            bool ok = true;
            while (((*tw - 1) * stride + KW) * ((*th - 1) * stride + KW) > conv_max_halo_slots(v)) {
                if (*tw > 1) *tw >>= 1; else if (*th > 1) *th >>= 1; else { ok = false; break; }
            }
            if (!ok) continue;
            *u = v;
            return true;
        }
        return false;
    };
    auto blocks = [&](const ConvTile& u, int tw, int th) {
        return B * (Wout / tw) * (Hout / th) * ((N + u.BN - 1) / u.BN);
    };
    const int bn_pref = N <= 32 ? 32 : (N <= 64 ? 64 : 128);
    const int bms[3] = {256, 128, 64};
    std::vector<int> bns = {bn_pref};
    if (bn_pref > 64) bns.push_back(64);
    long long best_blocks = -1;
    TileChoice best;
    bool found = false;
    for (int pass = 0; pass < 3 && best_blocks < 0; ++pass) {
        if (pass == 2) bns = {32, 64, 128};
        for (int bi = 0; bi < 3 && !found; ++bi)
            for (size_t ni = 0; ni < bns.size() && !found; ++ni) {
                ConvTile u;
                int tw, th;
                if (!pick(bms[bi], bns[ni], &u, &tw, &th)) continue;
                if (pass == 0 && tw * th * 2 <= u.BM && bi < 2 && !(stride == 2 && bi == 0)) continue;
                const long long nb = blocks(u, tw, th);
                if (nb > best_blocks) {
                    best_blocks = nb;
                    best.tile = u;
                    best.TW = tw;
                    best.TH = th;
                }
                if (nb >= ((taps == 1 && gn) ? 128 : 200)) found = true;
            }
    }
    if (g_force_bm && g_force_bn) {
        ConvTile u;
        int tw, th;
        if (pick(g_force_bm, g_force_bn, &u, &tw, &th)) {
            best.tile = u;
            best.TW = tw;
            best.TH = th;
            best_blocks = blocks(u, tw, th);
        }
    }
    c = best;
    if (best_blocks < 0) {
        c.tile.BM = 64; c.tile.BN = 64; c.tile.CK = 16; c.tile.taps = taps;
        return c;
    }
    c.ksplit = 1;
    const int ncc = Cin_pad / c.tile.CK;
    if (!nchw && g_force_ks > 0 && g_force_ks <= std::max(1, ncc)) c.ksplit = g_force_ks;
    return c;
}

struct Builder {
    Plan* plan;
    bool dry;
    Arena arena;
    int next_id = 0;
    std::map<int, int> refs;
    std::map<int, Tensor> live;
    char* base = nullptr;
    int launches = 0;
    int temb_ld = 0;
    int* ticket_ptr = nullptr;
    int tickets = 0;
    ViewPlan* vp = nullptr;
    bool recording = false;
    int conv_ord = 0;
    int groups_hint = 32;
    std::map<const NormParams*, Tensor> view_tensors;
    const std::vector<ViewPlan::Emit>* cur_emit = nullptr;

    void record_consumer(const NormParams* n, const Tensor& x0, const Tensor& x1, int silu, bool ok, int groups, float eps) {
        if (!vp || !recording || !n) return;
        ViewPlan::Cons c;
        c.parts.push_back({x0.prod, 0});
        if (x1.valid()) c.parts.push_back({x1.prod, x0.C});
        c.Ctot = x0.C + (x1.valid() ? x1.C : 0);
        c.silu = silu;
        c.groups = groups;
        c.eps = eps;
        c.ok = ok && x0.W * x0.H == (x1.valid() ? x1.W * x1.H : x0.W * x0.H);
        vp->cons[n] = c;
    }
    bool take_view(const NormParams* n, Tensor* v) {
        if (!vp || recording || !n) return false;
        auto it = vp->cons.find(n);
        if (it == vp->cons.end() || !it->second.use) return false;
// ... 362 lines not shown
                           (taps == 1 && Cin_t == 256) ? TK_CL_1x1_256 : -1;
        const int ranks_c = cluster_ranks(x0.B, N, Wout * Hout);
        const bool in_cluster = !in_trunk && cluster_enabled() && !a.own_image && kind_c >= 0 && BN == 64 && px_t == 64 &&
                                (p.up == 1 || p.up == 2) && vts.empty() && ranks_c == (N / 64) * p.tiles_img &&
                                p.Win * p.up == Wout && p.Hin * p.up == Hout;
        if (preact) {
            const bool gn_phase = gn_phase_t || (in_cluster && Cin_t <= 512 && (Wout * Hout) % ranks_c == 0 && a.x0.C % 8 == 0 &&
                                                 (!a.x1.valid() || a.x1.C % 8 == 0));
            if (gn_phase_t) trunk_begin(x0.B, ranks_t);
            else if (gn_phase) trunk_begin(x0.B, ranks_c, N / 64, 2);
            else note_launch();
            if (!dry) {
                GnApplyParams g;
                memset(&g, 0, sizeof(g));
                g.x0 = tptr(a.x0); g.x1 = tptr(a.x1);
                g.C0 = a.x0.C; g.C1 = a.x1.valid() ? a.x1.C : 0;
                g.st0 = sptr(a.x0); g.st1 = sptr(a.x1);
                g.P0 = a.x0.P; g.P1 = a.x1.valid() ? a.x1.P : 0;
                g.B = a.x0.B; g.npix = a.x0.W * a.x0.H;
                g.groups = a.groups;
                g.gamma = a.gn->gamma.as<float>(); g.beta = a.gn->beta.as<float>();
                g.eps = a.eps; g.silu = a.silu;
                g.y = tptr(act);
                const double by = (double)g.B * g.npix * Cin_t * 4.0;
                if (gn_phase) {
                    g.inv_n = (float)(1.0 / ((double)g.npix * (Cin_t / g.groups)));
                    pend.phases.push_back(trunk_gn_apply_phase(g));
                    pend.lds = std::max(pend.lds, (size_t)(2 * 512 * 8 + 2 * 512 * 4));
                    pend.bytes += by;
                }
                emit({[g](hipStream_t st) { return launch_gn_apply(g, st); }, "gn_apply_kernel", 0.0, by}, gn_phase);
            }
        }
        if (in_trunk) trunk_begin(x0.B, ranks_t);
        else if (in_cluster) trunk_begin(x0.B, ranks_c, N / 64, 2);
        else note_launch();
        in_trunk = in_trunk || in_cluster;
        if (!dry) {
            ConvLayer::Packed* pk = nullptr;
            if (L->get_fragpacked(Cin_t, BN == 16 ? 16 : 32, BN == 16 ? 8 : conv_small_kgroups(BN), epi_res, &pk)) return 1;
            ConvArgs k = a;
            k.x0 = x0;
            if (!gn_fused) k.gn = nullptr;
            if (!gn_fused || p.C1 == 0) k.x1 = Tensor();
            if (epi_res) {
                p.res = tptr(a.r0);
                k.r0 = k.r1 = Tensor();
            }
            bind_conv(p, k, *pk, y);
            for (size_t v = 0; v < vts.size(); ++v) {
                const auto& e = (*cur_emit)[v];
                NormView& nv = p.nv[v];
                nv.y = tptr(vts[v]) + e.ch_off;
                nv.gamma = e.norm->gamma.as<float>() + e.ch_off;
                nv.beta = e.norm->beta.as<float>() + e.ch_off;
                nv.ld = e.Ctot;
                const int cpg = e.Ctot / e.groups;
                nv.cpg_shift = 0;
                while ((1 << nv.cpg_shift) < cpg) ++nv.cpg_shift;
                nv.inv_n = (float)(1.0 / ((double)Wout * Hout * cpg));
                nv.eps = e.eps;
                nv.silu = e.silu;
            }
            p.nviews = (int)vts.size();
            Plan* pl = plan;
            const int temb_off = a.temb_off;
            const double by = conv_bytes(a, s, 1 + vts.size());
            const std::string kname = "conv_small_kernel<" + std::to_string(p.TW * p.TH) + "," + std::to_string(BN) + ",taps" + std::to_string(taps) + ">";
            if (in_trunk) {
                RLDM_REQUIRE(!in_cluster || p.nviews == 0, "conv " + L->name + ": a multi-tile cluster phase writes no views");
                TrunkPhase ph = trunk_conv_phase(p, in_cluster ? kind_c : trunk_kind, in_cluster, temb_off);
                const int KG = in_cluster ? 4 : 8, ksc = BN == 16 ? 32 : 16, cpt = Cin_t / (ksc * KG);
                int G;
                if (in_cluster) G = (taps == 1 ? 1 : (cpt <= 2 ? 9 : (cpt <= 4 ? 3 : 1))) * cpt;
                else G = BN == 16 ? (taps == 9 ? 9 : 1) * cpt : ((trunk_kind & 3) == 0 ? 18 : ((trunk_kind & 3) == 1 ? 12 : cpt));
                ph.w[TW_G] = std::min(G, kTrunkPrefetch);
                ph.w[TW_NMINE] = taps * cpt + ((p.R0 + p.R1) / ksc) / KG;
                ph.w[TW_WBYTES] = (unsigned)((N / (in_cluster ? 32 : BN)) * KG * ph.w[TW_NMINE]) * 1024u;
                pend.phases.push_back(ph);
                pend.lds = std::max(pend.lds, conv_small_lds_bytes(p, taps, BN));
                pend.flops += fl;
                pend.bytes += by;
            }
            const ConvLate late{temb_off};
            emit({[p, BN, taps, pl, late](hipStream_t st) mutable {
                late.apply(p, pl->io);
                return launch_conv_small(p, taps, BN, st);
            }, kname, fl, by}, in_trunk);
        }
        if (preact) release(act);
        *out = y;
        return 0;
    }

    static constexpr int kSubMinBlocks = 96;
    static constexpr long long kAnyGrid = 1ll << 40;
    static bool stream_params_tw(const ConvArgs& a, const ConvShape& s, StreamInst inst, long long min_blocks, long long max_blocks,
                                 ConvParams* q, StreamTile tile = {}) {
        const StreamInstDesc& d = kStreamInst[inst];
        if (tile.TW == 0) tile = d.tiles[0];
        const int TW = tile.TW, TH = tile.TH;
        if (dbg() & RLDM_FLAG_NO_STREAM_REGW) return false;
        if (s.taps != 9 || a.stride != d.STR || a.pad_mode != 0 || a.out_f32_nchw || g_force_bm) return false;
        const bool sub = d.SUB;
        ConvShape tiled = s;
        if (sub) {
            if (a.up != 2 || s.R_t != 0 || s.Wout != 2 * a.x0.W || s.Hout != 2 * a.x0.H) return false;
            tiled.Wout = a.x0.W; tiled.Hout = a.x0.H;
        }
        if (tiled.Wout % TW != 0 || tiled.Hout % TH != 0) return false;
        conv_geometry(a, tiled, TW, TH, d.FH ? TH : (TH - 1) * a.stride + 3, q);
        if (sub) {
            q->up = 1;
            q->Wout = s.Wout; q->Hout = s.Hout;
        }
        q->st_inst = inst;
        ConvTile t;
        t.BM = 256; t.BN = 128; t.CK = 64; t.taps = 9;
        q->colb = conv_halo_col_bytes(t, TH, a.stride);
        const long long blocks = (long long)q->B * q->tiles_img * (q->N / d.bn()) * (sub ? 4 : 1);
        return supported_with(*q, a.gn != nullptr, false, [](const ConvParams& c) { return conv_stream_supported(c, 9); }) &&
               ((dbg() & RLDM_FLAG_STREAM_ANY_GRID) || (blocks >= min_blocks && blocks <= max_blocks));
    }
    static bool stream_params(const ConvArgs& a, const ConvShape& s, ConvParams* q) {
        const int R_t = s.R_t, Hout = s.Hout;
        const auto fits = [&](StreamInst inst, long long min_blocks, long long max_blocks, StreamTile tile = {}) {
            return stream_params_tw(a, s, inst, min_blocks, max_blocks, q, tile);
        };
        const int N_ = a.layer->Cout;
        const bool n128 = N_ % 128 == 0;
        if (a.stride == 2) {
            if (!n128 || R_t != 0 || a.up != 1) return false;
            if (fits(SI_64x128_S2, kInst4MinBlocks, 512, {8, 8})) return true;
            return Hout == 4 && fits(SI_64x128_S2, 48, 512, {16, 4});
        }
        const int f2 = dbg2();
        const StreamInst px256 = n128 ? SI_256x128 : SI_256x64;
        if ((f2 & RLDM_FLAG2_STREAM_SPEC_WAVES) && n128 && fits(SI_256x128_SPEC, 200, kAnyGrid)) return true;
        if ((f2 & RLDM_FLAG2_STREAM_64PX) && n128 && fits(SI_64x128, 192, 512)) return true;
        if (!(f2 & RLDM_FLAG2_STREAM_8WAVE_FULL) && a.up == 2 && n128 &&
            (fits(SI_SUB_W4, kSubMinBlocks, kAnyGrid) || (a.x0.H % 8 != 0 && fits(SI_SUB_T4_W4, kSubMinBlocks, kAnyGrid)))) return true;
        if (!(f2 & (RLDM_FLAG2_STREAM_8WAVE_FULL | RLDM_FLAG2_HALO_RING)) && n128 && (Hout == 16 || Hout == 8) && a.up == 1 &&
            fits(SI_FULLH_W4, 384, kAnyGrid, {Hout == 16 ? 8 : 16, Hout})) return true;
        if (!(f2 & RLDM_FLAG2_STREAM_8WAVE_FULL) && n128 && fits(SI_128x128_W4, 384, kAnyGrid)) return true;
        if (!(f2 & RLDM_FLAG2_STREAM_8WAVE_C64) && !n128 && fits(SI_128x64_W4, 384, kAnyGrid)) return true;
        if (fits(px256, 200, kAnyGrid)) return true;
        if (n128 && Hout == 8 && fits(SI_64x128, kInst4MinBlocks, 320)) return true;
        if (!(f2 & RLDM_FLAG2_STREAM_8WAVE_128X8) && fits(SI_128x64_W4, 257, 512)) return true;
        if (fits(SI_128x64, 128, 512, {16, 8})) return true;
        if (Hout % 8 != 0 && fits(SI_128x64, 128, 512, {32, 4})) return true;
        return fits(px256, 128, kAnyGrid);
    }

    int conv_stream(const ConvArgs& a, const ConvShape& s, ConvParams p, Tensor* out) {
        ConvLayer* L = a.layer;
        const int N = L->Cout;
        const Tensor& x0 = a.x0;
        if (require_gn_input(a, s.Cin_t)) return 1;
        p.dbg = kernel_dbg();
        p.ts = stamp_buf(StampSite::Conv, conv_ord - 1);
        const StreamInstDesc& d = stream_inst(p);
        const bool sub = d.SUB;
        p.ntile_n = N / d.bn() * (sub ? 4 : 1);
        Tensor y = make(x0.B, s.Wout, s.Hout, N);
        if (a.want_stats) add_stats(y, p.tiles_img * (sub ? 4 : 1));
        const double fl_ref = conv_flops(a, s);
        plan->flops += fl_ref;
        const double fl = sub ? fl_ref * 4.0 / 9.0 : fl_ref;
        const int ranks_s = p.tiles_img * p.ntile_n;
        const int per_cu = d.wg_per_cu();
        const bool in_stream_cluster = cluster_enabled() && ranks_s >= 2 && ranks_s <= 16 * per_cu &&
                                       trunk_grid_fits(ranks_s, x0.B, per_cu) && y.P <= kFoldAboveP && N % 128 == 0 &&
                                       d.trunk != TSF_NONE && (!sub || N == 128) && conv_stream_lds_bytes(p) <= (size_t)d.lds_cap();
        if (in_stream_cluster) trunk_begin(x0.B, ranks_s, sub ? 1 : p.ntile_n, 4, d.NW == 4 ? 4 : 2);
        else note_launch();
        if (!dry) {
            ConvLayer::Packed* pk = nullptr;
            if (sub ? L->get_subpixpacked(s.Cin_t, &pk) : L->get_streampacked(s.Cin_t, d.kgroups(), &pk)) return 1;
            bind_conv(p, a, *pk, y);
            Plan* pl = plan;
            const int temb_off = a.temb_off;
            const double by = conv_bytes(a, s);
            if (in_stream_cluster) {
                pend.phases.push_back(trunk_conv_phase(p, TK_STREAM, true, temb_off));
                pend.lds = std::max(pend.lds, conv_stream_lds_bytes(p));
                pend.flops += fl;
                pend.bytes += by;
            }
            const ConvLate late{temb_off};
            emit({[p, pl, late](hipStream_t st) mutable {
                late.apply(p, pl->io);
                return launch_conv_stream(p, st);
            }, "conv_stream_kernel<" + std::to_string(p.TW * p.TH) + "," + std::to_string(d.bn()) + ",CK64,taps9" + (p.stride == 2 ? ",s2" : "") + (sub ? ",sub" : "") + ">", fl, by}, in_stream_cluster);
        }
        *out = y;
        return 0;
    }

    static bool c16_params(const ConvArgs& a, const ConvShape& s, ConvParams* q) {
        const int Cin_t = s.Cin_t, R_t = s.R_t, taps = s.taps, Wout = s.Wout, Hout = s.Hout;
        if ((dbg() & RLDM_FLAG_NO_STREAM_REGW) || g_force_bm || taps != 9 || a.stride != 1 || a.pad_mode != 0 || a.up != 1 || a.out_f32_nchw) return false;
        if (a.x1.valid() || a.gn || a.temb_off >= 0 || R_t != 0 || Cin_t != 16 || a.layer->Cout % 128 != 0 || Wout % 16 != 0 || Hout % 8 != 0) return false;
        conv_geometry(a, s, 16, 8, 0, q);
        q->ntile_n = q->N / 128;
        return conv_c16_supported(*q) && (long long)q->B * q->tiles_img * q->ntile_n >= 64;
    }
    int conv_c16(const ConvArgs& a, const ConvShape& s, ConvParams p, Tensor* out) {
        Tensor y = make(a.x0.B, s.Wout, s.Hout, a.layer->Cout);
        if (a.want_stats) add_stats(y, p.tiles_img);
        const double fl = conv_flops(a, s);
        plan->flops += fl;
        note_launch();
        if (!dry) {
            ConvLayer::Packed* pk = nullptr;
            if (a.layer->get_c16packed(&pk)) return 1;
            bind_conv(p, a, *pk, y);
            Plan* pl = plan;
            const ConvLate late{-1, a.first_of_step};
            emit({[p, pl, late](hipStream_t st) mutable {
                late.apply(p, pl->io);
                return launch_conv_c16(p, st);
            }, "conv_c16_kernel<128,128,taps9>", fl, conv_bytes(a, s)});
        }
        *out = y;
        return 0;
    }

    static bool o4_params(const ConvArgs& a, const ConvShape& s, ConvParams* q) {
        const int Cin_t = s.Cin_t, R_t = s.R_t, taps = s.taps, Wout = s.Wout, Hout = s.Hout;
        if ((dbg() & RLDM_FLAG_NO_STREAM_REGW) || g_force_bm || taps != 9 || a.stride != 1 || a.pad_mode != 0 || a.up != 1 || !a.out_f32_nchw) return false;
        if (a.x1.valid() || a.temb_off >= 0 || R_t != 0 || Cin_t != 128 || a.layer->Cin != 128 || a.layer->Cout > 4 || Wout % 16 != 0 || Hout % 8 != 0) return false;
        conv_geometry(a, s, 16, 8, 0, q);
        q->ntile_n = 1;
        return supported_with(*q, a.gn != nullptr, true, conv_o4_supported) && (long long)q->B * q->tiles_img >= 64;
    }
    int conv_o4(const ConvArgs& a, const ConvShape& s, ConvParams p, Tensor* out) {
        if (require_gn_input(a, s.Cin_t)) return 1;
        const double fl = conv_flops(a, s);
        plan->flops += fl;
        note_launch();
        if (!dry) {
            ConvLayer::Packed* pk = nullptr;
            if (a.layer->get_streampacked(128, 2, &pk)) return 1;
            bind_conv(p, a, *pk, Tensor());
            Plan* pl = plan;
            const ConvLate late{-1, false, true, true};
            emit({[p, pl, late](hipStream_t st) mutable {
                late.apply(p, pl->io);
                return launch_conv_o4(p, st);
            }, "conv_o4_kernel<128,32,taps9>", fl, conv_bytes(a, s)});
        }
        *out = Tensor();
        return 0;
    }

    static bool ds2_params(const ConvArgs& a, const ConvShape& s, ConvParams* q) {
        const int Cin_t = s.Cin_t, R_t = s.R_t, taps = s.taps, Wout = s.Wout;
        if ((dbg() & RLDM_FLAG_NO_STREAM_REGW) || g_force_bm || taps != 9 || a.stride != 2 || a.pad_mode != 0 || a.up != 1 || a.out_f32_nchw) return false;
        if (a.x1.valid() || a.gn || a.temb_off >= 0 || R_t != 0 || Cin_t != 256 || a.layer->Cin != 256 || a.layer->Cout % 32 != 0 || Wout % 32 != 0) return false;
        conv_geometry(a, s, 32, 1, 0, q);
        q->ntile_n = q->N / 32;
        const long long blocks = (long long)q->B * q->tiles_img * q->ntile_n;
        return conv_ds2_supported(*q) && blocks >= 32 && blocks <= 512;
    }
    int conv_ds2(const ConvArgs& a, const ConvShape& s, ConvParams p, Tensor* out) {
        Tensor y = make(a.x0.B, s.Wout, s.Hout, a.layer->Cout);
        if (a.want_stats) add_stats(y, p.tiles_img);
        const double fl = conv_flops(a, s);
        plan->flops += fl;
        note_launch();
        if (!dry) {
            ConvLayer::Packed* pk = nullptr;
            if (a.layer->get_streampacked(256, 2, &pk)) return 1;
            bind_conv(p, a, *pk, y);
            emit({[p](hipStream_t st) { return launch_conv_ds2(p, st); }, "conv_ds2_kernel<32,32,taps9,s2>", fl, conv_bytes(a, s)});
        }
        *out = y;
        return 0;
    }

    static bool regw_params(const ConvArgs& a, const ConvShape& s, ConvParams* q) {
        const int N_ = a.layer->Cout, Cin_t = s.Cin_t, R_t = s.R_t, taps = s.taps, Wout = s.Wout, Hout = s.Hout;
        if ((dbg2() & RLDM_FLAG2_NO_REGW) || (dbg() & RLDM_FLAG_NO_STREAM_REGW) || g_force_bm || taps != 9 || a.stride != 1 || a.pad_mode != 0 || a.up != 1) return false;
        if (a.x1.valid() || a.temb_off >= 0 || Cin_t != 64 || a.layer->Cin != 64 || a.first_of_step) return false;
        if (a.out_f32_nchw ? (N_ > 4 || R_t != 0) : N_ != 64) return false;
        if (R_t != 0 && !(a.layer->sc_identity && R_t == 64 && a.r0.valid() && a.r0.C == 64)) return false;
        if (Wout % 16 != 0 || Hout % 8 != 0) return false;
        conv_geometry(a, s, 16, 8, 10, q);
        ConvTile t;
        t.BM = 256; t.BN = 128; t.CK = 64; t.taps = 9;
        q->colb = conv_halo_col_bytes(t, 8, 1);
        q->exp = (dbg2() & RLDM_FLAG2_REGW_CAP8) ? 8 : 0;
        return supported_with(*q, a.gn != nullptr, a.out_f32_nchw, conv_regw_supported);
    }
    int conv_regw(const ConvArgs& a, const ConvShape& s, ConvParams p, Tensor* out) {
        if (require_gn_input(a, s.Cin_t)) return 1;
        p.dbg = kernel_dbg();
        p.ts = g_ts_buf;
        p.ntile_n = 1;
        Tensor y;
        if (!a.out_f32_nchw) {
            y = make(a.x0.B, s.Wout, s.Hout, a.layer->Cout);
            if (a.want_stats) add_stats(y, conv_regw_partials(p));
        }
        const double fl = conv_flops(a, s);
        plan->flops += fl;
        note_launch();
        if (!dry) {
            ConvLayer::Packed* pk = nullptr;
            if (a.layer->get_streampacked(s.Cin_t, 1, &pk)) return 1;
            bind_conv(p, a, *pk, y);
            Plan* pl = plan;
            const ConvLate late{-1, false, a.out_f32_nchw};
            emit({[p, pl, late](hipStream_t st) mutable {
                RLDM_REQUIRE(!late.f32_out || pl->io.sch.coef_table == nullptr, "conv_regw: a scheduler step fused into this output layer");
                late.apply(p, pl->io);
                return launch_conv_regw(p, st);
            }, std::string("conv_regw_kernel<128,") + (late.f32_out ? "32" : "64") + ",taps9>", fl, conv_bytes(a, s, 1, false)});
        }
        *out = y;
        return 0;
    }

    static constexpr int kFoldAboveP = 32;
    int fold_stats(Tensor& y) {
        if (!y.valid() || y.P <= kFoldAboveP) return 0;
        const size_t raw_off = y.st_off, raw_bytes = y.st_bytes();
        const int rawP = y.P;
        add_stats(y, 2);
        note_launch();
        if (!dry) {
            GnFoldParams g;
            g.part = ptr<float2>(raw_off);
            g.out = ptr<float2>(y.st_off);
            g.B = y.B; g.P = rawP; g.C = y.C;
            plan->ops.push_back({[g](hipStream_t s) { return launch_gn_fold(g, s); }, "gn_fold_kernel", 0.0, (double)raw_bytes});
        }
        arena.release(raw_off, raw_bytes);
        return 0;
    }

    int conv(const ConvArgs& a0, Tensor* out) {
        ConvArgs a = a0;
        const int ord = conv_ord++;
        ConvLayer* L = a.layer;
        RLDM_REQUIRE(L != nullptr, "internal: missing conv layer");
// ... 1736 lines not shown
        const float* noise = s->cfg.mode == RLDM_SAMPLER_DDPM ? step_noise + lat_off : nullptr;
        ln->guided = GuidedIO();
        if (s->cfg.guided) {
            ln->guided.known = gio.known + lat_off;
            ln->guided.mask = gio.mask + (size_t)ln->b0 * s->unet->cfg.sample_w * s->unet->cfg.sample_h;
            ln->guided.known_noise = gio.known_noise ? gio.known_noise + lat_off : nullptr;
            ln->guided.renoise_noise = gio.renoise_noise ? gio.renoise_noise + lat_off : nullptr;
        }
        if (!ln->step_graph || ln->captured_noise != noise || !(ln->captured_guided == ln->guided)) {
            if (sampler_enqueue_step(s, ln, noise, st)) return 1;
            RLDM_HIP_CHECK(hipStreamSynchronize(st));
            if (ln->uplan->trunk_error.p) {
                int terr = 0;
                RLDM_HIP_CHECK(hipMemcpy(&terr, ln->uplan->trunk_error.p, 4, hipMemcpyDeviceToHost));
                const bool off = ((g_dbg_flags | s->plan_flags) & RLDM_FLAG_NO_PERSISTENT) != 0;
                if (getenv("RLDM_TEST_TRUNK_FAIL") && !off) terr = 2;
                if (terr != 0 && !off) {
                    if (sampler_drop_persistent(s, "persistent launches failed their self-check at the warm-up step", terr)) return 1;
                    return sample_impl(s, x_T, step_noise, cond, gio, images, latents_out, stream);
                }
                RLDM_REQUIRE(terr == 0, "persistent trunk launch failed its self-check (code " + std::to_string(terr) +
                                            "): set RLDM_DBG_FLAGS=16777216 to run the levels as separate launches");
            }
            RLDM_HIP_CHECK(hipMemcpyAsync(ln->x.p, x_T + lat_off, ln->n_latent * 4, hipMemcpyDeviceToDevice, st));
            if (sampler_pack_x(s, ln, st)) return 1;
            if (launch_step_counter(ln->step.as<int>(), ln->fused_tail ? -1 : 0, 0, st)) return 1;
            int gs = std::max(1, std::min(kGraphSteps, s->cfg.num_steps));
            while (s->cfg.num_steps % gs != 0) --gs;
            ln->graph_steps = gs;
            if (capture(st, [&]() {
                    for (int k = 0; k < gs; ++k)
                        if (sampler_enqueue_step(s, ln, noise, st)) return 1;
                    return 0;
                }, &ln->step_graph)) return 1;
            ln->captured_noise = noise;
            ln->captured_guided = ln->guided;
        }
        if (images && s->vae && !ln->decode_graph) {
            if (ln->dplan->run(st)) return 1;
            RLDM_HIP_CHECK(hipStreamSynchronize(st));
            if (capture(st, [&]() { return ln->dplan->run(st); }, &ln->decode_graph)) return 1;
            RLDM_HIP_CHECK(hipMemcpyAsync(ln->x.p, x_T + lat_off, ln->n_latent * 4, hipMemcpyDeviceToDevice, st));
            if (sampler_pack_x(s, ln, st)) return 1;
        }
    }
    if (s->inject_error) {
        for (auto& lnp : s->lanes)
            if (lnp->uplan->trunk_error.p && launch_step_counter(lnp->uplan->trunk_error.as<int>(), s->inject_error, 0, lnp->stream)) return 1;
        s->inject_error = 0;
    }
    for (int i = 0; i < s->cfg.num_steps; i += s->lanes[0]->graph_steps)
        for (auto& lnp : s->lanes) RLDM_HIP_CHECK(hipGraphLaunch(lnp->step_graph, lnp->stream));
    for (auto& lnp : s->lanes) {
        SamplerLane* ln = lnp.get();
        hipStream_t st = ln->stream;
        const size_t lat_off = (size_t)ln->b0 * (ln->n_latent / ln->nb);
        if (latents_out)
            RLDM_HIP_CHECK(hipMemcpyAsync(latents_out + lat_off, ln->x.p, ln->n_latent * 4, hipMemcpyDeviceToDevice, st));
        if (images) {
            if (s->vae) {
                RLDM_HIP_CHECK(hipGraphLaunch(ln->decode_graph, st));
                RLDM_HIP_CHECK(hipMemcpyAsync(images + (size_t)ln->b0 * (ln->n_image / ln->nb), ln->image.p, ln->n_image * 4,
                                              hipMemcpyDeviceToDevice, st));
            } else {
                RLDM_HIP_CHECK(hipMemcpyAsync(images + lat_off, ln->x.p, ln->n_latent * 4, hipMemcpyDeviceToDevice, st));
            }
        }
        if (ln->uplan->trunk_error.p) {
            if (!ln->check_host) {
                RLDM_HIP_CHECK(hipHostMalloc(reinterpret_cast<void**>(&ln->check_host), 64, hipHostMallocDefault));
                *ln->check_host = 0;
            }
            float* img_l = images ? images + (s->vae ? (size_t)ln->b0 * (ln->n_image / ln->nb) : lat_off) : nullptr;
            if (launch_trunk_check(ln->uplan->trunk_error.as<int>(), img_l, s->vae ? ln->n_image : ln->n_latent,
                                   latents_out ? latents_out + lat_off : nullptr, ln->n_latent, st)) return 1;
            RLDM_HIP_CHECK(hipMemcpyAsync(ln->check_host, ln->uplan->trunk_error.p, 4, hipMemcpyDeviceToHost, st));
            ln->check_pending = true;
        }
        RLDM_HIP_CHECK(hipEventRecord(ln->ev_out, st));
        ln->call_recorded = true;
        RLDM_HIP_CHECK(hipStreamWaitEvent(caller, ln->ev_out, 0));
    }
    return 0;
}

int rldm_sample(rldm_sampler* s, const float* x_T, const float* step_noise, const float* cond, float* images,
                float* latents_out, void* stream) {
    RLDM_REQUIRE(s, "null argument");
    RLDM_REQUIRE(!s->cfg.guided, "this sampler was created with guided = 1: call rldm_sample_guided (known, mask and the two noise "
                                 "tensors are part of every row)");
    return sample_impl(s, x_T, step_noise, cond, GuidedIO(), images, latents_out, stream);
}

int rldm_sample_guided(rldm_sampler* s, const float* x_T, const float* step_noise, const float* known, const float* mask,
                       const float* known_noise, const float* renoise_noise, float* images, float* latents_out, void* stream) {
    RLDM_REQUIRE(s, "null argument");
    RLDM_REQUIRE(s->cfg.guided, "rldm_sample_guided needs a sampler created with guided = 1");
    RLDM_REQUIRE(known && mask, "null argument: known / mask");
    RLDM_REQUIRE(known_noise || !s->needs_known_noise, "some row has kb != 0: known_noise must be given");
    RLDM_REQUIRE(renoise_noise || !s->needs_renoise_noise, "some row jumps back up: renoise_noise must be given");
    GuidedIO gio;
    gio.known = known; gio.mask = mask; gio.known_noise = known_noise; gio.renoise_noise = renoise_noise;
    return sample_impl(s, x_T, step_noise, nullptr, gio, images, latents_out, stream);
}

int rldm_sampler_profile(rldm_sampler* s, const float* x_T, char* json_out, size_t cap) {
    RLDM_REQUIRE(s && x_T && json_out && cap > 2, "null argument");
    SamplerLane* ln = s->lanes[0].get();
    hipStream_t st = ln->stream;
    RLDM_HIP_CHECK(hipMemcpyAsync(ln->x.p, x_T, ln->n_latent * 4, hipMemcpyDeviceToDevice, st));
    if (sampler_pack_x(s, ln, st)) return 1;
    if (launch_step_counter(ln->step.as<int>(), ln->fused_tail ? -1 : 0, 0, st)) return 1;
    if (ln->uplan->run(st)) return 1;
    RLDM_HIP_CHECK(hipStreamSynchronize(st));
    std::map<std::string, KernelStat> unet_stats, vae_stats;
    if (ln->uplan->run_profiled(st, unet_stats)) return 1;
    if (ln->dplan) {
        if (ln->dplan->run(st)) return 1;
        RLDM_HIP_CHECK(hipStreamSynchronize(st));
        if (ln->dplan->run_profiled(st, vae_stats)) return 1;
    }
    std::string js = "{";
    auto dump = [&](const char* key, const std::map<std::string, KernelStat>& m) {
        js += std::string("\"") + key + "\": {";
        bool first = true;
        for (auto& kv : m) {
            if (!first) js += ", ";
            first = false;
            char buf[512];
            snprintf(buf, sizeof(buf), "\"%s\": {\"launches\": %d, \"ms\": %.6f, \"flops\": %.6e, \"bytes\": %.6e}",
                     kv.first.c_str(), kv.second.launches, kv.second.ms, kv.second.flops, kv.second.bytes);
            js += buf;
        }
        js += "}";
    };
    dump("unet_step", unet_stats);
    js += ", ";
    dump("vae_decode", vae_stats);
    js += ", \"plan_flags\": " + std::to_string(s->plan_flags) + ", \"fell_back\": " + (s->plan_flags != s->cfg.plan_flags ? "true" : "false");
    js += ", \"lanes\": " + std::to_string(s->lanes.size()) + ", \"lane_batch\": " + std::to_string(ln->nb) + "}";
    RLDM_REQUIRE(js.size() + 1 <= cap, "profile buffer too small");
    memcpy(json_out, js.c_str(), js.size() + 1);
    return 0;
}

namespace {
struct ConvCase {
    Layers layers;
    Plan plan;
    Tensor t0, t1, tr, out;
    int Wout = 0, Hout = 0, C0p = 0;
};
int make_conv_case(ConvCase& cc, const rldm_conv_desc* d, const float* weight, const float* bias, const float* gamma,
                   const float* beta, int res_channels, bool with_temb) {
    const bool with_res = res_channels > 0;
    const int Cin = d->Cin0 + d->Cin1;
    cc.C0p = d->Cin1 ? d->Cin0 : pad16(d->Cin0);
    RLDM_REQUIRE(d->Cin1 == 0 || (d->Cin0 % 16 == 0 && Cin % 16 == 0), "concat test needs Cin0 % 16 == 0 and Cin % 16 == 0");
    ParamStore ps;
    ps.host["c.weight"].assign(weight, weight + (size_t)d->Cout * Cin * d->ksize * d->ksize);
    ps.host["c.bias"].assign(bias, bias + d->Cout);
    if (cc.layers.add_conv(ps, "c", d->Cout, Cin, d->ksize)) return 1;
    if (with_res) {
        ConvLayer* L = cc.layers.get_conv("c");
        L->R = res_channels;
        L->sc_identity = res_channels == d->Cout;
        if (!L->sc_identity) {
            L->sc_w.resize((size_t)d->Cout * res_channels);
            uint32_t rng = 777u;
            for (auto& v : L->sc_w) {
                rng = rng * 1664525u + 1013904223u;
                v = (((rng >> 8) & 0xffff) / 32768.0f - 1.0f) / std::sqrt((float)res_channels);
            }
        }
    }
    if (d->gn) {
        RLDM_REQUIRE(gamma && beta && cc.C0p + d->Cin1 == Cin, "GroupNorm test needs unpadded channels");
        ps.host["n.weight"].assign(gamma, gamma + Cin);
        ps.host["n.bias"].assign(beta, beta + Cin);
        if (cc.layers.add_norm(ps, "n", Cin)) return 1;
    }
    const int s = d->stride, up = d->upsample ? 2 : 1;
    cc.Wout = d->Win * up / s;
    cc.Hout = d->Hin * up / s;
    auto walk = [&cc, d, with_res, res_channels, with_temb, s, up](Builder& bb) -> int {
        cc.t0 = bb.make(d->B, d->Win, d->Hin, cc.C0p);
        cc.t1 = Tensor();
        cc.tr = Tensor();
        if (d->Cin1) cc.t1 = bb.make(d->B, d->Win, d->Hin, d->Cin1);
        if (with_res) cc.tr = bb.make(d->B, cc.Wout, cc.Hout, res_channels);
        if (d->gn) {
            if (bb.gn_stats(cc.t0)) return 1;
            if (d->Cin1 && bb.gn_stats(cc.t1)) return 1;
        }
        ConvArgs a;
        a.layer = cc.layers.get_conv("c");
        a.x0 = cc.t0; a.x1 = cc.t1;
        a.stride = s; a.pad_mode = d->pad_mode; a.up = up;
        a.gn = d->gn ? cc.layers.get_norm("n") : nullptr;
        a.eps = d->eps; a.silu = d->silu;
        a.temb_off = with_temb ? 0 : -1;
        a.r0 = cc.tr;
        a.want_stats = true;
        if ((dbg2() & RLDM_FLAG2_FP32_OUT) && d->Cout <= 4 && !with_res && !with_temb) {
            a.out_f32_nchw = true;
            a.want_stats = false;
        }
        return bb.conv(a, &cc.out);
    };
    return build_plan(&cc.plan, d->Cout, walk);
}
}

int rldm_test_conv(const rldm_conv_desc* d, const float* x0, const float* x1, const float* weight, const float* bias,
                   const float* gamma, const float* beta, const float* temb, const float* res, float* y, void* stream) {
    RLDM_REQUIRE(d && x0 && weight && bias && y, "null argument");
    hipStream_t st = reinterpret_cast<hipStream_t>(stream);
    ConvCase cc;
    if (make_conv_case(cc, d, weight, bias, gamma, beta, res ? d->Cout : 0, temb != nullptr)) return 1;
    DevBuf tembd;
    if (temb && upload(tembd, temb, (size_t)d->B * d->Cout * 4)) return 1;
    char* base = cc.plan.arena.as<char>();
    auto tp = [&](const Tensor& t) { return reinterpret_cast<bf16_t*>(base + t.off); };
    if (launch_nchw_f32_to_nhwc_bf16(x0, tp(cc.t0), d->B, d->Cin0, d->Win, d->Hin, cc.C0p, st)) return 1;
    if (d->Cin1 && launch_nchw_f32_to_nhwc_bf16(x1, tp(cc.t1), d->B, d->Cin1, d->Win, d->Hin, d->Cin1, st)) return 1;
    if (res && launch_nchw_f32_to_nhwc_bf16(res, tp(cc.tr), d->B, d->Cout, cc.Wout, cc.Hout, d->Cout, st)) return 1;
    cc.plan.io.temb = tembd.as<float>();
    cc.plan.io.temb_rows_per_step = d->B;
    cc.plan.io.temb_per_sample = 1;
    if (!cc.out.valid()) cc.plan.io.out = y;
    if (cc.plan.run(st)) return 1;
    if (cc.out.valid() && launch_nhwc_bf16_to_nchw_f32(tp(cc.out), y, d->B, d->Cout, cc.Wout, cc.Hout, d->Cout, st)) return 1;
    RLDM_HIP_CHECK(hipStreamSynchronize(st));
    return 0;
}

int rldm_test_conv_stats(const rldm_conv_desc* d, const float* x0, const float* weight, const float* bias, float* stats,
                         void* stream) {
    RLDM_REQUIRE(d && x0 && weight && bias && stats, "null argument");
    RLDM_REQUIRE(d->Cin1 == 0 && !d->gn, "stats test: plain single-input conv only");
    hipStream_t st = reinterpret_cast<hipStream_t>(stream);
    ConvCase cc;
    if (make_conv_case(cc, d, weight, bias, nullptr, nullptr, 0, false)) return 1;
    char* base = cc.plan.arena.as<char>();
    if (launch_nchw_f32_to_nhwc_bf16(x0, reinterpret_cast<bf16_t*>(base + cc.t0.off), d->B, d->Cin0, d->Win, d->Hin, cc.C0p, st)) return 1;
    if (cc.plan.run(st)) return 1;
    RLDM_HIP_CHECK(hipStreamSynchronize(st));
    RLDM_REQUIRE(cc.out.P > 0, "internal: conv output carries no statistics");
    std::vector<float2> part((size_t)d->B * cc.out.P * d->Cout);
    RLDM_HIP_CHECK(hipMemcpy(part.data(), base + cc.out.st_off, part.size() * sizeof(float2), hipMemcpyDeviceToHost));
    std::vector<float> hs((size_t)d->B * d->Cout * 2, 0.f);
    for (int b = 0; b < d->B; ++b)
        for (int q = 0; q < cc.out.P; ++q)
            for (int c = 0; c < d->Cout; ++c) {
                const float2 v = part[((size_t)b * cc.out.P + q) * d->Cout + c];
                hs[((size_t)b * d->Cout + c) * 2] += v.x;
                hs[((size_t)b * d->Cout + c) * 2 + 1] += v.y;
            }
    RLDM_HIP_CHECK(hipMemcpy(stats, hs.data(), hs.size() * 4, hipMemcpyHostToDevice));
    return 0;
}

int rldm_debug_set_flags2(int flags) {
    g_dbg_flags2 = flags;
    return 0;
}
int rldm_debug_set_flags(int flags) {
    g_dbg_flags = flags;
    return 0;
}

static constexpr int kTsBlocks = 2048;
int rldm_debug_timestamps(unsigned long long* host_out) {
    if (!g_ts_buf) {
        RLDM_HIP_CHECK(hipMalloc(reinterpret_cast<void**>(&g_ts_buf), (256 + 2 * kTsBlocks) * 8));
        RLDM_HIP_CHECK(hipMemset(g_ts_buf, 0, (256 + 2 * kTsBlocks) * 8));
    }
    if (host_out) {
        RLDM_HIP_CHECK(hipDeviceSynchronize());
        RLDM_HIP_CHECK(hipMemcpy(host_out, g_ts_buf, 256 * 8, hipMemcpyDeviceToHost));
        RLDM_HIP_CHECK(hipMemset(g_ts_buf, 0, 256 * 8));
    }
    return 0;
}
int rldm_debug_block_times(unsigned long long* host_out, int nblocks) {
    RLDM_REQUIRE(host_out && nblocks >= 1 && nblocks <= kTsBlocks, "block times: 1..2048 blocks");
    RLDM_REQUIRE(g_ts_buf != nullptr, "block times: call rldm_debug_timestamps(NULL) first");
    RLDM_HIP_CHECK(hipDeviceSynchronize());
    RLDM_HIP_CHECK(hipMemcpy(host_out, g_ts_buf + 256, (size_t)nblocks * 16, hipMemcpyDeviceToHost));
    RLDM_HIP_CHECK(hipMemset(g_ts_buf + 256, 0, 2 * kTsBlocks * 8));
    return 0;
}

int rldm_debug_graph_trace(unsigned long long* stamps, int cap, char* names, size_t names_cap) {
    if (!g_trace.p || !g_trace_plan) return 0;
    (void)hipDeviceSynchronize();
    int n = 0;
    for (auto& o : g_trace_plan->ops) n += (!o.active || o.active()) ? 1 : 0;
    const int m = std::min(cap, n + 1);
    if (stamps && m > 0 && hipMemcpy(stamps, g_trace.p, (size_t)m * 8, hipMemcpyDeviceToHost) != hipSuccess) return -1;
    if (names && names_cap) {
        std::string all;
        for (auto& o : g_trace_plan->ops)
            if (!o.active || o.active()) all += o.name + "\n";
        strncpy(names, all.c_str(), names_cap - 1);
        names[names_cap - 1] = 0;
    }
    return n;
}

int rldm_debug_force_tile(int BM, int BN, int ksplit) {
    g_force_bm = BM;
    g_force_bn = BN;
    g_force_ks = ksplit;
    return 0;
}

int rldm_bench_conv(const rldm_conv_desc* d, int with_res, int with_temb, int warmup, int iters, float* avg_us,
                    char* kernel_name, size_t name_cap, void* stream) {
    RLDM_REQUIRE(d && avg_us && iters >= 1, "bad argument");
    hipStream_t st = reinterpret_cast<hipStream_t>(stream);
    const int Cin = d->Cin0 + d->Cin1;
    const int taps = d->ksize * d->ksize;
    std::vector<float> w((size_t)d->Cout * Cin * taps), bias(d->Cout), gamma(Cin, 1.f), beta(Cin, 0.f);
    uint32_t rng = 12345u;
    auto rnd = [&]() { rng = rng * 1664525u + 1013904223u; return ((rng >> 8) & 0xffff) / 32768.0f - 1.0f; };
    const float ws = 1.0f / std::sqrt((float)Cin * taps);
    for (auto& v : w) v = rnd() * ws;
    for (auto& v : bias) v = rnd() * 0.1f;
    ConvCase cc;
    if (make_conv_case(cc, d, w.data(), bias.data(), gamma.data(), beta.data(), with_res, with_temb != 0)) return 1;
    DevBuf tembd;
    if (with_temb) {
        std::vector<float> t((size_t)d->B * d->Cout);
        for (auto& v : t) v = rnd();
        if (upload(tembd, t.data(), t.size() * 4)) return 1;
    }
    {
        std::vector<bf16_t> h(cc.plan.arena.bytes / 2);
        for (auto& v : h) v = f32_to_bf16(rnd());
        RLDM_HIP_CHECK(hipMemcpy(cc.plan.arena.p, h.data(), h.size() * 2, hipMemcpyHostToDevice));
    }
    cc.plan.io.temb = tembd.as<float>();
    cc.plan.io.temb_rows_per_step = d->B;
    cc.plan.io.temb_per_sample = 1;
    DevBuf outd;
    if (!cc.out.valid()) {
        if (outd.alloc((size_t)d->B * d->Cout * cc.Wout * cc.Hout * sizeof(float))) return 1;
        cc.plan.io.out = outd.as<float>();
    }
    RLDM_REQUIRE(!cc.plan.ops.empty(), "internal: empty plan");
    size_t last = cc.plan.ops.size() - 1;
    while (last > 0 && cc.plan.ops[last].name.rfind("conv_", 0) != 0) --last;
    size_t first = last;
    if (first > 0 && cc.plan.ops[first - 1].name == "gn_apply_kernel") --first;
    auto run_unit = [&]() {
        for (size_t o = first; o <= last; ++o)
            if (cc.plan.ops[o].fn(st)) return 1;
        return 0;
    };
    if (kernel_name && name_cap) {
        const std::string nm = (first < last ? "gn_apply+" : "") + cc.plan.ops[last].name;
        strncpy(kernel_name, nm.c_str(), name_cap - 1);
        kernel_name[name_cap - 1] = 0;
    }
    if (cc.plan.run(st)) return 1;
    for (int i = 0; i < warmup; ++i)
        if (run_unit()) return 1;
    hipEvent_t e0, e1;
    RLDM_HIP_CHECK(hipEventCreate(&e0));
    RLDM_HIP_CHECK(hipEventCreate(&e1));
    RLDM_HIP_CHECK(hipEventRecord(e0, st));
    for (int i = 0; i < iters; ++i)
        if (run_unit()) return 1;
    RLDM_HIP_CHECK(hipEventRecord(e1, st));
    RLDM_HIP_CHECK(hipStreamSynchronize(st));
    float ms = 0.f;
    RLDM_HIP_CHECK(hipEventElapsedTime(&ms, e0, e1));
    (void)hipEventDestroy(e0);
    (void)hipEventDestroy(e1);
    *avg_us = ms * 1000.0f / iters;
    return 0;
}

int rldm_test_attention(const float* qkv, int B, int L, int C, float* out, void* stream) {
    RLDM_REQUIRE(qkv && out, "null argument");
// ... 208 lines not shown
```

Baseline: 256.5 range-images/sec.

## Add persistent multi-tile streaming conv kernel for large tile counts

Adds a persistent variant of the streaming implicit-GEMM conv. A fixed number of workgroups (CUs times workgroups per CU) each walk a contiguous range of output tiles, and the next tile's halo and weights are prefetched while the current tile's epilogue runs. This is meant to remove per-tile workgroup launch and prologue cost and the wave-quantization tail when tiles far outnumber slots. It applies only when there are at least four tiles per slot and outside stream clusters. It adds a large new kernel body and a raw-conv test entry point, and it risks register pressure and LDS aliasing limits.

```diff
diff --git a/include/rangeldm_hip.h b/include/rangeldm_hip.h
--- a/include/rangeldm_hip.h
+++ b/include/rangeldm_hip.h
@@ -433,6 +433,9 @@
 } rldm_conv_desc;
 int rldm_test_conv(const rldm_conv_desc* d, const float* x0, const float* x1, const float* weight, const float* bias,
                    const float* gamma, const float* beta, const float* temb, const float* res, float* y, void* stream);
+int rldm_test_conv_raw(const rldm_conv_desc* d, const void* x0, const void* x1, const float* weight, const float* bias,
+                       const float* gamma, const float* beta, const void* res, void* st0, void* st1, void* y, void* y_stats,
+                       const int* parts, char* kernel_name, size_t name_cap, void* stream);
 int rldm_bench_conv(const rldm_conv_desc* d, int with_res, int with_temb, int warmup, int iters, float* avg_us,
                     char* kernel_name, size_t name_cap, void* stream);
 int rldm_debug_force_tile(int BM, int BN, int ksplit);
@@ -454,9 +457,11 @@
     RLDM_FLAG_OWN_IMAGE_COPIES = 1 << 22,
     RLDM_FLAG_SCHED_LAUNCH     = 1 << 23,
     RLDM_FLAG_NO_PERSISTENT    = 1 << 24,
-    RLDM_FLAG_NO_CLUSTERS      = 1 << 26
+    RLDM_FLAG_NO_CLUSTERS      = 1 << 26,
+    RLDM_FLAG_NO_STREAM_MULTITILE = 1 << 27
 };
 int rldm_debug_set_flags(int flags);
+int rldm_debug_stream_multitile_cap(int wgs);
 enum rldm_flag2 {
     RLDM_FLAG2_STREAM_8WAVE_FULL = 1,
     RLDM_FLAG2_STREAM_8WAVE_128X8 = 2,
diff --git a/rangeldm_amd/_lib.py b/rangeldm_amd/_lib.py
--- a/rangeldm_amd/_lib.py
+++ b/rangeldm_amd/_lib.py
@@ -30,6 +30,7 @@
     SCHED_LAUNCH = 1 << 23
     NO_PERSISTENT = 1 << 24
     NO_CLUSTERS = 1 << 26
+    NO_STREAM_MULTITILE = 1 << 27
 
 
 class Flag2(enum.IntFlag):
@@ -286,6 +287,8 @@
     "rldm_unet_trunk_status": (C.c_int, [_P, C.c_int]),
     "rldm_sampler_profile": (C.c_int, [_P, _P, C.c_char_p, C.c_size_t]),
     "rldm_test_conv": (C.c_int, [C.POINTER(ConvDescC), _P, _P, _P, _P, _P, _P, _P, _P, _P, _P]),
+    "rldm_test_conv_raw": (C.c_int, [C.POINTER(ConvDescC)] + [_P] * 11 + [C.POINTER(C.c_int), C.c_char_p, C.c_size_t, _P]),
+    "rldm_debug_stream_multitile_cap": (C.c_int, [C.c_int]),
     "rldm_bench_conv": (C.c_int, [C.POINTER(ConvDescC), C.c_int, C.c_int, C.c_int, C.c_int, C.POINTER(C.c_float),
                                   C.c_char_p, C.c_size_t, _P]),
     "rldm_debug_force_tile": (C.c_int, [C.c_int, C.c_int, C.c_int]),
diff --git a/rangeldm_amd/csrc/conv_stream.hip b/rangeldm_amd/csrc/conv_stream.hip
--- a/rangeldm_amd/csrc/conv_stream.hip
+++ b/rangeldm_amd/csrc/conv_stream.hip
@@ -1,4 +1,5 @@
 #include "conv_stream_body.h"
+#include "conv_stream_multi_body.h"
 #include "conv_stream_spec_body.h"
 
 #include <utility>
@@ -21,6 +22,16 @@
     conv_stream_body<WM, WN, false, NW, MI, S, SUB, T4, FH>(p, nt, mt, b, none);
 }
 
+template <int WN, bool SUB, bool FH>
+__global__ void __launch_bounds__(256, 2) conv_stream_multi_kernel(const ConvParams p) {
+    const int nwg = p.mt_wgs;
+    const long long total = (long long)p.ntile_n * p.tiles_img * p.B;
+    const int w = xcd_remap(blockIdx.x, nwg);
+    const int t0 = (int)(w * total / nwg), t1 = (int)((w + 1) * total / nwg);
+    if (t0 >= t1) return;
+    conv_stream_multi_body<WN, SUB, FH>(p, t0, t1);
+}
+
 __global__ void __launch_bounds__(512, 1) conv_stream_spec_kernel(const ConvParams p) {
     int nt, mt, b;
     {
@@ -40,14 +51,25 @@
 int conv_stream_kgroups(const ConvParams& p) { return stream_inst(p).kgroups(); }
 int conv_stream_threads(const ConvParams& p) { return stream_inst(p).threads(); }
 
-size_t conv_stream_lds_bytes(const ConvParams& p) {
+static size_t stream_halo_bytes(const ConvParams& p) { return (size_t)2 * ((p.TW - 1) * p.stride + 3) * p.colb; }
+static size_t stream_alias_bytes(const ConvParams& p) {
     const int BN = conv_stream_bn(p), KG = conv_stream_kgroups(p), BM = p.TW * p.TH;
-    const size_t a = (size_t)((p.TW - 1) * p.stride + 3) * p.colb;
-    const size_t main_bytes = 2 * a + (size_t)(p.C0 + p.C1) * 8 + BN * 4;
     const size_t gscratch = p.st0 ? (size_t)2 * (p.C0 + p.C1) * 8 : 0;
     const size_t epi = KG == 1 ? (size_t)BM * (BN * 2 + 16) + (size_t)8 * 2 * BN * 4
                                : (size_t)KG * 64 * (BN * 4 + 16) + (size_t)64 * (BN * 2 + 16) + (size_t)8 * 2 * BN * 4;
-    return std::max(std::max(main_bytes, gscratch), epi);
+    return std::max(gscratch, epi);
+}
+
+size_t conv_stream_lds_bytes(const ConvParams& p) {
+    const size_t main_bytes = stream_halo_bytes(p) + (size_t)(p.C0 + p.C1) * 8 + conv_stream_bn(p) * 4;
+    return std::max(main_bytes, stream_alias_bytes(p));
+}
+
+bool conv_stream_multi_supported(const ConvParams& p) {
+    if (p.st_inst < 0 || p.st_inst >= SI_COUNT) return false;
+    const StreamInstDesc& d = stream_inst(p);
+    if (d.spec || d.NW != 4 || d.MI != 4 || d.STR != 1 || d.T4) return false;
+    return stream_alias_bytes(p) <= stream_halo_bytes(p);
 }
 
 bool conv_stream_supported(const ConvParams& p, int taps) {
@@ -72,6 +94,18 @@
     void (*kern)(const ConvParams);
     if constexpr (d.spec) kern = conv_stream_spec_kernel;
     else kern = conv_stream_kernel<d.WM, d.WN, d.NW, d.MI, d.STR, d.SUB, d.T4, d.FH>;
+    if constexpr (!d.spec && d.NW == 4 && d.MI == 4 && d.STR == 1 && !d.T4) {
+        if (p.mt_wgs > 0) {
+            RLDM_REQUIRE(conv_stream_multi_supported(p), "conv_stream: no multi-tile form for this shape");
+            void (*multi)(const ConvParams) = conv_stream_multi_kernel<d.WN, d.SUB, d.FH>;
+            static DynLdsLimit multi_lds_limit;
+            RLDM_HIP_CHECK(multi_lds_limit.ensure(reinterpret_cast<const void*>(multi), lds));
+            hipLaunchKernelGGL(multi, dim3(p.mt_wgs), dim3(d.threads()), lds, stream, p);
+            RLDM_HIP_CHECK(hipGetLastError());
+            return 0;
+        }
+    }
+    RLDM_REQUIRE(p.mt_wgs == 0, "conv_stream: this instance has no multi-tile form");
     static DynLdsLimit lds_limit;
     RLDM_HIP_CHECK(lds_limit.ensure(reinterpret_cast<const void*>(kern), lds));
     hipLaunchKernelGGL(kern, dim3(p.N / d.bn() * (d.SUB ? 4 : 1), p.tiles_img, p.B), dim3(d.threads()), lds, stream, p);
diff --git a/rangeldm_amd/csrc/conv_stream_multi_body.h b/rangeldm_amd/csrc/conv_stream_multi_body.h
--- /dev/null
+++ b/rangeldm_amd/csrc/conv_stream_multi_body.h
@@ -0,0 +1,545 @@
+#pragma once
+#include "conv_stream_body.h"
+
+namespace rldm {
+
+struct StreamTileId {
+    int nt, par_w, par_h;
+    int b, mt, w0, h0;
+};
+
+template <int WN, bool SUB, bool FH>
+__device__ __forceinline__ void conv_stream_multi_body(const ConvParams& p, const int t_first, const int t_end) {
+    static_assert(WN == 4 || (WN == 2 && !SUB && !FH), "the 4-wave instances: 128 x 128 (plain, sub-pixel, full-height) and 128 x 64");
+    constexpr int TAPW = SUB ? 2 : 3;
+    constexpr StreamInstDesc D = {1, WN, 4, 4};
+    constexpr int NT = D.threads(), CK = 64, KG = D.kgroups(), NW = 4, MI = 4;
+    constexpr int BM = D.bm(), BN = D.bn();
+    constexpr int RS = CK * 2 + 16, C8 = CK / 8;
+    constexpr int HALO_PX = FH ? (8 + 2) * 16 : (16 + 2) * 10;
+    constexpr int ACH = (HALO_PX * C8 + NT - 1) / NT;
+    constexpr int SPT = 4 / KG, ROW = TAPW * SPT, CST = TAPW * TAPW * SPT;
+    constexpr int G = ROW;
+    constexpr int PFX = KG == 1 ? 2 : 3;
+    constexpr int ERS = BN * 2 + 16, NC8 = BN / 8;
+    constexpr int CPT = 512 / NT;
+    static_assert(KG <= 2 && CST % PFX == 0 && CST % G == 0 && PFX <= ROW, "wave grid");
+    extern __shared__ __attribute__((aligned(16))) unsigned char smem[];
+    const int wave = __builtin_amdgcn_readfirstlane(threadIdx.x >> 6);
+    const int kg = wave / WN, wn = wave % WN;
+    int tid, lane, kh, l31, my_c8;
+    unsigned woff;
+    int xoff[4];
+
+    const int gx = p.ntile_n, gy = p.tiles_img, tiles_h = p.tiles_h;
+    const int th_log = 31 - __builtin_clz(tiles_h);
+    auto tile_of = [&](int rid) __attribute__((always_inline)) {
+        StreamTileId t;
+        const int q = rid / gx, nt_ = rid - q * gx;
+        t.b = q / gy;
+        t.mt = q - t.b * gy;
+        t.nt = SUB ? nt_ >> 2 : nt_;
+        t.par_w = SUB ? (nt_ >> 1) & 1 : 0;
+        t.par_h = SUB ? nt_ & 1 : 0;
+        t.w0 = (t.mt >> th_log) * p.TW;
+        t.h0 = (t.mt & (tiles_h - 1)) * p.TH;
+        return t;
+    };
+    const int Cin = p.C0 + p.C1;
+    const int NCC = Cin / CK, NCB = (p.R0 + p.R1) / CK, NCT = NCC + NCB;
+    const int THv = p.TH + 2, TWv = p.TW + 2;
+    const int colb = p.colb;
+    const int abytes = TWv * colb;
+    const int Wv = p.Win * p.up, Hv = p.Hin * p.up;
+    const int upshift = p.up - 1;
+    unsigned char* sA = smem;
+    float* sGa = reinterpret_cast<float*>(sA + 2 * abytes);
+    float* sGs = sGa + Cin;
+    float* sBias = sGs + Cin;
+    const int nsteps = NCC * CST + NCB * SPT;
+    auto w_load = [&](const unsigned char* base, int idx) __attribute__((always_inline)) {
+        return *reinterpret_cast<const bf16x8*>(base + (idx / 8) * 8192 + woff + ((idx % 8) * 1024 - 4096));
+    };
+    auto w_stream = [&](const StreamTileId& t) __attribute__((always_inline)) {
+        return reinterpret_cast<const unsigned char*>(p.wpk) +
+               (size_t)(SUB ? (t.nt * WN + wn) * 4 + (t.par_w * 2 + t.par_h) : (t.nt * WN + wn) * KG + kg) * nsteps * 1024;
+    };
+    const int THs = FH ? p.TH : THv;
+    const int atotal = TWv * THs * C8;
+    const bool gn = p.st0 != nullptr;
+    const bf16_t* const gx0 = p.x0;
+    const bf16_t* const gx1 = p.x1;
+    const bf16_t* const gr0 = p.r0;
+    const bf16_t* const gr1 = p.r1;
+    const int nC0 = p.C0, nC1 = p.C1, nR0 = p.R0, nR1 = p.R1;
+    auto rederive = [&]() __attribute__((always_inline)) {
+        tid = threadIdx.x;
+        asm volatile("" : "+v"(tid));
+        lane = tid & 63;
+        kh = lane >> 5;
+        l31 = lane & 31;
+        my_c8 = (tid % C8) * 8;
+        woff = lane * 16 + 4096;
+#pragma unroll
+        for (int mi = 0; mi < MI; ++mi) {
+            const int pidx = mi * 32 + l31;
+            const int pw = pidx >> p.th_shift, ph = pidx - (pw << p.th_shift);
+            xoff[mi] = pw * colb + ph * RS + kh * 16 + kg * (SPT * 32);
+        }
+    };
+    rederive();
+    const int temb_step = (p.temb && p.step_ptr && tid < BN) ? load_step_vector(p.step_ptr) : 0;
+
+    StreamTileId cur = tile_of(t_first);
+    int apix[ACH];
+    uint4 areg[ACH];
+    bf16x8 wr[G];
+    const unsigned char* wptr;
+    float bias_v = 0.f;
+    auto load_a = [&](int cs) __attribute__((always_inline)) {
+        const int c = cs * CK + my_c8;
+        const bool first = c < nC0;
+        const bf16_t* base = first ? gx0 + c : gx1 + (c - nC0);
+        const int ld = first ? nC0 : nC1;
+#pragma unroll
+        for (int i = 0; i < ACH; ++i) {
+            const int pix = apix[i] < 0 ? 0 : apix[i];
+            areg[i] = ld_act16(base + (size_t)pix * ld);
+        }
+    };
+    auto store_a = [&](int cs) __attribute__((always_inline)) {
+        unsigned char* dstbuf = sA + (cs & 1) * abytes;
+        float4 ga0, ga1, gs0, gs1;
+        if (gn) {
+            const int c = cs * CK + my_c8;
+            ga0 = *reinterpret_cast<const float4*>(sGa + c);
+            ga1 = *reinterpret_cast<const float4*>(sGa + c + 4);
+            gs0 = *reinterpret_cast<const float4*>(sGs + c);
+            gs1 = *reinterpret_cast<const float4*>(sGs + c + 4);
+        }
+#pragma unroll
+        for (int i = 0; i < ACH; ++i) {
+            uint4 v = areg[i];
+            if (apix[i] < 0) {
+                v = make_uint4(0u, 0u, 0u, 0u);
+            } else if (gn) {
+                float f0 = bf16lo(v.x) * ga0.x + gs0.x, f1 = bf16hi(v.x) * ga0.y + gs0.y;
+                float f2 = bf16lo(v.y) * ga0.z + gs0.z, f3 = bf16hi(v.y) * ga0.w + gs0.w;
+                float f4 = bf16lo(v.z) * ga1.x + gs1.x, f5 = bf16hi(v.z) * ga1.y + gs1.y;
+                float f6 = bf16lo(v.w) * ga1.z + gs1.z, f7 = bf16hi(v.w) * ga1.w + gs1.w;
+                if (p.silu) {
+                    silu_x8(f0, f1, f2, f3, f4, f5, f6, f7);
+                }
+                v.x = pack_bf16x2(f0, f1); v.y = pack_bf16x2(f2, f3);
+                v.z = pack_bf16x2(f4, f5); v.w = pack_bf16x2(f6, f7);
+            }
+            const int q = tid + i * NT;
+            const int slot = q / C8, c8 = q - slot * C8;
+            const int vwl = (slot * p.magic_thv) >> 20, vhl = slot - vwl * THs + (FH ? 1 : 0);
+            if (q < atotal) *reinterpret_cast<uint4*>(dstbuf + vwl * colb + vhl * RS + c8 * 16) = v;
+        }
+    };
+    constexpr int RCH = (BM * C8 + NT - 1) / NT;
+    static_assert(RCH <= ACH && (BM * C8) % NT == 0, "residual pieces fit the halo registers");
+    constexpr int RSTEP = NT / C8;
+    auto load_r = [&](int cs, uint4* rr) __attribute__((always_inline)) {
+        const int cb = (cs - NCC) * CK;
+        const bool first = cb < nR0;
+        const bf16_t* base = (first ? gr0 + cb : gr1 + (cb - nR0)) + my_c8;
+        const int ld = first ? nR0 : nR1;
+        const int pidx = tid / C8, pw = pidx >> p.th_shift, ph = pidx - (pw << p.th_shift);
+        const bf16_t* src = base + (size_t)((cur.b * p.Wout + cur.w0 + pw) * p.Hout + cur.h0 + ph) * ld;
+        const size_t step = (size_t)((RSTEP >> p.th_shift) * p.Hout) * ld;
+#pragma unroll
+        for (int i = 0; i < RCH; ++i) rr[i] = ld_act16(src + i * step);
+    };
+    auto store_r = [&](int cs, const uint4* rr) __attribute__((always_inline)) {
+        const int pidx = tid / C8, pw = pidx >> p.th_shift, ph = pidx - (pw << p.th_shift);
+        unsigned char* dst = sA + (cs & 1) * abytes + (pw + 1) * colb + (ph + 1) * RS + (tid % C8) * 16;
+        const int step = (RSTEP >> p.th_shift) * colb;
+#pragma unroll
+        for (int i = 0; i < RCH; ++i) *reinterpret_cast<uint4*>(dst + i * step) = rr[i];
+    };
+    auto request = [&](const StreamTileId& t) __attribute__((always_inline)) {
+#pragma unroll
+        for (int i = 0; i < ACH; ++i) {
+            const int q = tid + i * NT;
+            const int slot = q / C8;
+            const int vwl = (slot * p.magic_thv) >> 20, vhl = slot - vwl * THs + (FH ? 1 : 0);
+            const int vh = t.h0 - 1 + vhl;
+            int vw = t.w0 - 1 + vwl;
+            vw = vw < 0 ? vw + Wv : (vw >= Wv ? vw - Wv : vw);
+            const bool ok = q < atotal && vh >= 0 && vh < Hv;
+            apix[i] = ok ? ((t.b * p.Win + (vw >> upshift)) * p.Hin + (vh >> upshift)) : -1;
+        }
+        if (NCT > 0) load_a(0);
+        const unsigned char* ws = w_stream(t);
+#pragma unroll
+        for (int j = 0; j < G; ++j) {
+            wr[j] = w_load(ws, j);
+            __builtin_amdgcn_sched_barrier(0);
+        }
+        wptr = ws + G * 1024;
+        bias_v = 0.f;
+        if (tid < BN) {
+            bias_v = p.bias[t.nt * BN + tid];
+            if (p.temb) bias_v += p.temb[(size_t)(temb_step * p.temb_rows_per_step + (p.temb_per_sample ? t.b : 0)) * p.temb_ld + t.nt * BN + tid];
+        }
+    };
+    double gS[CPT], gSS[CPT];
+    float g_gamma[CPT], g_beta[CPT];
+    auto fold_load = [&](int b) __attribute__((always_inline)) {
+#pragma unroll
+        for (int sl = 0; sl < CPT; ++sl) {
+            gS[sl] = 0.0; gSS[sl] = 0.0; g_gamma[sl] = 0.f; g_beta[sl] = 0.f;
+            const int ch = tid + sl * NT;
+            if (ch < Cin) {
+                const bool first = ch < nC0;
+                const int c = first ? ch : ch - nC0;
+                const int C = first ? nC0 : nC1;
+                const int P = first ? p.P0 : p.P1;
+                const float2* src = (first ? p.st0 : p.st1) + (size_t)b * P * C + c;
+                g_gamma[sl] = p.gn_gamma[ch];
+                g_beta[sl] = p.gn_beta[ch];
+                int q = 0;
+                for (; q + 32 <= P; q += 32) {
+                    float2 v[32];
+#pragma unroll
+                    for (int j = 0; j < 32; ++j) v[j] = ld_act8(src + (size_t)(q + j) * C);
+#pragma unroll
+                    for (int j = 0; j < 32; ++j) { gS[sl] += (double)v[j].x; gSS[sl] += (double)v[j].y; }
+                }
+                for (; q + 16 <= P; q += 16) {
+                    float2 v[16];
+#pragma unroll
+                    for (int j = 0; j < 16; ++j) v[j] = ld_act8(src + (size_t)(q + j) * C);
+#pragma unroll
+                    for (int j = 0; j < 16; ++j) { gS[sl] += (double)v[j].x; gSS[sl] += (double)v[j].y; }
+                }
+                for (; q + 4 <= P; q += 4) {
+                    float2 v[4];
+#pragma unroll
+                    for (int j = 0; j < 4; ++j) v[j] = ld_act8(src + (size_t)(q + j) * C);
+#pragma unroll
+                    for (int j = 0; j < 4; ++j) { gS[sl] += (double)v[j].x; gSS[sl] += (double)v[j].y; }
+                }
+                for (; q < P; ++q) {
+                    const float2 v = ld_act8(src + (size_t)q * C);
+                    gS[sl] += (double)v.x;
+                    gSS[sl] += (double)v.y;
+                }
+            }
+        }
+    };
+    auto fold_finish = [&]() __attribute__((always_inline)) {
+        double* sD = reinterpret_cast<double*>(sA);
+        const int cpg = Cin / p.gn_groups;
+#pragma unroll
+        for (int sl = 0; sl < CPT; ++sl) {
+            const int ch = tid + sl * NT;
+            if (ch < Cin) {
+                sD[ch] = gS[sl];
+                sD[Cin + ch] = gSS[sl];
+            }
+        }
+        __syncthreads();
+        float ga[CPT], gs[CPT];
+#pragma unroll
+        for (int sl = 0; sl < CPT; ++sl) {
+            const int ch = tid + sl * NT;
+            ga[sl] = 0.f; gs[sl] = 0.f;
+            if (ch < Cin) {
+                const int g0 = ((ch * p.magic_cpg) >> 20) * cpg;
+                double S = 0.0, SS = 0.0;
+                for (int i = 0; i < cpg; ++i) {
+                    S += sD[g0 + i];
+                    SS += sD[Cin + g0 + i];
+                }
+                const double inv_n = (double)p.gn_inv_n;
+                const double mean = S * inv_n;
+                double var = SS * inv_n - mean * mean;
+                var = var < 0.0 ? 0.0 : var;
+                ga[sl] = g_gamma[sl] * __builtin_amdgcn_rsqf((float)var + p.gn_eps);
+                gs[sl] = g_beta[sl] - (float)mean * ga[sl];
+            }
+        }
+#pragma unroll
+        for (int sl = 0; sl < CPT; ++sl) {
+            const int ch = tid + sl * NT;
+            if (ch < Cin) {
+                sGa[ch] = ga[sl];
+                sGs[ch] = gs[sl];
+            }
+        }
+        __syncthreads();
+    };
+
+    int b_folded = -1;
+    if (gn) fold_load(cur.b);
+    request(cur);
+    if (gn) {
+        fold_finish();
+        b_folded = cur.b;
+    }
+
+    for (int t = t_first;; ++t) {
+        if (t != t_first) rederive();
+        if (gn && cur.b != b_folded) {
+            fold_load(cur.b);
+            fold_finish();
+            b_folded = cur.b;
+        }
+        if (tid < BN) sBias[tid] = bias_v;
+        if constexpr (FH) {
+            const int nz = TWv * 2 * 2 * (RS / 16);
+            for (int q = tid; q < nz; q += NT) {
+                const int sl = q % (RS / 16), r = q / (RS / 16);
+                const int col = r >> 2, which = r & 3;
+                *reinterpret_cast<uint4*>(sA + (which >> 1) * abytes + col * colb + ((which & 1) ? (THv - 1) * RS : 0) + sl * 16) = make_uint4(0u, 0u, 0u, 0u);
+            }
+        }
+        if (NCT > 0) store_a(0);
+        const int paroff = cur.par_w * colb + cur.par_h * RS;
+        lds_barrier_b();
+        f32x16 acc[MI];
+#pragma unroll
+        for (int r4 = 0; r4 < 4; ++r4) {
+            float4 bv = *reinterpret_cast<const float4*>(sBias + wn * 32 + 8 * r4 + 4 * kh);
+            if (kg != 0) bv = make_float4(0.f, 0.f, 0.f, 0.f);
+#pragma unroll
+            for (int mi = 0; mi < MI; ++mi) {
+                acc[mi][r4 * 4 + 0] = bv.x; acc[mi][r4 * 4 + 1] = bv.y;
+                acc[mi][r4 * 4 + 2] = bv.z; acc[mi][r4 * 4 + 3] = bv.w;
+            }
+        }
+
+        bf16x8 xr[PFX][MI];
+        auto x_read = [&](const int (&cr)[MI], const int (&nx)[MI], int r, bf16x8 (&dst)[MI]) __attribute__((always_inline)) {
+#pragma unroll
+            for (int mi = 0; mi < MI; ++mi)
+                dst[mi] = *reinterpret_cast<const bf16x8*>(smem + (r < ROW ? cr[mi] : nx[mi]) + ((r % ROW) / SPT) * RS + (r % SPT) * 32);
+        };
+        auto tap_row = [&](const int (&cr)[MI], const int (&nx)[MI], int ti) __attribute__((always_inline)) {
+#pragma unroll
+            for (int j = 0; j < ROW; ++j) {
+                const int c = ti * ROW + j, slot = c % G;
+#pragma unroll
+                for (int mi = 0; mi < MI; ++mi) {
+                    acc[mi] = __builtin_amdgcn_mfma_f32_32x32x16_bf16(wr[slot], xr[c % PFX][mi], acc[mi], 0, 0, 0);
+                    if (c + PFX < CST) {
+                        const int r = j + PFX;
+                        xr[c % PFX][mi] = *reinterpret_cast<const bf16x8*>(smem + (r < ROW ? cr[mi] : nx[mi]) + ((r % ROW) / SPT) * RS + (r % SPT) * 32);
+                    }
+                }
+                wr[slot] = w_load(wptr, slot);
+#pragma unroll
+                for (int mi = 0; mi < MI; ++mi) {
+                    __builtin_amdgcn_sched_group_barrier(0x008, 1, 0);
+                    if (c + PFX < CST) __builtin_amdgcn_sched_group_barrier(0x100, 1, 0);
+                }
+                __builtin_amdgcn_sched_group_barrier(0x020, 1, 0);
+                __builtin_amdgcn_sched_barrier(0);
+            }
+            if ((ti * ROW + ROW) % G == 0) wptr += G * 1024;
+        };
+        for (int cs = 0; cs < NCC; ++cs) {
+            if (cs + 1 < NCT) {
+                if (cs + 1 < NCC) load_a(cs + 1);
+                else load_r(cs + 1, areg);
+            }
+            int cr[MI], nx[MI];
+            const int boff = (cs & 1) * abytes + paroff;
+#pragma unroll
+            for (int mi = 0; mi < MI; ++mi) { cr[mi] = xoff[mi] + boff; nx[mi] = cr[mi] + colb; }
+#pragma unroll
+            for (int j = 0; j < PFX; ++j) {
+                x_read(cr, nx, j, xr[j]);
+                __builtin_amdgcn_sched_barrier(0);
+            }
+            tap_row(cr, nx, 0);
+            if (cs + 1 < NCT) {
+                if (cs + 1 < NCC) store_a(cs + 1);
+                else store_r(cs + 1, areg);
+            }
+#pragma unroll
+            for (int mi = 0; mi < MI; ++mi) { cr[mi] = nx[mi]; nx[mi] += colb; }
+            tap_row(cr, nx, 1);
+            if constexpr (TAPW == 3) {
+#pragma unroll
+                for (int mi = 0; mi < MI; ++mi) cr[mi] = nx[mi];
+                tap_row(cr, nx, 2);
+            }
+            lds_barrier_b();
+        }
+        constexpr int RCR = G / SPT;
+        uint4 rreg[RCH];
+        for (int rc0 = 0; rc0 < NCB; rc0 += RCR) {
+#pragma unroll
+            for (int r = 0; r < RCR; ++r) {
+                const int rc = rc0 + r;
+                if (rc < NCB) {
+                    const int cs = NCC + rc;
+                    if (rc + 1 < NCB) load_r(cs + 1, rreg);
+                    int xc[MI];
+#pragma unroll
+                    for (int mi = 0; mi < MI; ++mi) xc[mi] = xoff[mi] + (cs & 1) * abytes + colb + RS;
+#pragma unroll
+                    for (int ks = 0; ks < SPT; ++ks) {
+                        bf16x8 xf[MI];
+#pragma unroll
+                        for (int mi = 0; mi < MI; ++mi) xf[mi] = *reinterpret_cast<const bf16x8*>(smem + xc[mi] + ks * 32);
+#pragma unroll
+                        for (int mi = 0; mi < MI; ++mi)
+                            acc[mi] = __builtin_amdgcn_mfma_f32_32x32x16_bf16(wr[r * SPT + ks], xf[mi], acc[mi], 0, 0, 0);
+                        wr[r * SPT + ks] = w_load(wptr, r * SPT + ks);
+                    }
+                    if (rc + 1 < NCB) store_r(cs + 1, rreg);
+                    lds_barrier_b();
+                }
+                if (r == RCR - 1) wptr += G * 1024;
+            }
+        }
+
+        const bool more = t + 1 < t_end;
+        const StreamTileId done = cur;
+        rederive();
+        if (more) {
+            cur = tile_of(t + 1);
+            request(cur);
+        }
+
+        if constexpr (KG > 1) {
+            constexpr int HB = 64, NHALF = BM / HB, FRS = BN * 4 + 16, TRS = BN * 2 + 16;
+            constexpr int NPASS = (HB * NC8 + NT - 1) / NT;
+            unsigned char* sE = smem;
+            unsigned char* sT = sE + KG * HB * FRS;
+            const int c8 = tid % NC8;
+            const int chg = done.nt * BN + c8 * 8;
+            constexpr int NCP = BN / 2, NG = NT / NCP, PPG = HB / NG;
+            const int cp = tid % NCP, pg = tid / NCP;
+            float s0 = 0.f, s1 = 0.f, q0 = 0.f, q1 = 0.f;
+#pragma unroll
+            for (int hp = 0; hp < NHALF; ++hp) {
+                if (hp > 0) lds_barrier_b();
+#pragma unroll
+                for (int m2 = 0; m2 < 2; ++m2) {
+                    const int mi = (hp % 2) * 2 + m2, pl = m2 * 32 + l31;
+#pragma unroll
+                    for (int r4 = 0; r4 < 4; ++r4) {
+                        const int chl = wn * 32 + 8 * r4 + 4 * kh;
+                        *reinterpret_cast<float4*>(sE + (kg * HB + pl) * FRS + chl * 4) =
+                            make_float4(acc[mi][r4 * 4 + 0], acc[mi][r4 * 4 + 1], acc[mi][r4 * 4 + 2], acc[mi][r4 * 4 + 3]);
+                    }
+                }
+                lds_barrier_b();
+#pragma unroll
+                for (int q = 0; q < NPASS; ++q) {
+                    const int pl = tid / NC8 + q * (NT / NC8), pidx = hp * HB + pl;
+                    if (pl >= HB) break;
+                    float f[8] = {0.f, 0.f, 0.f, 0.f, 0.f, 0.f, 0.f, 0.f};
+#pragma unroll
+                    for (int g = 0; g < KG; ++g) {
+                        const float4 v0 = *reinterpret_cast<const float4*>(sE + (g * HB + pl) * FRS + c8 * 32);
+                        const float4 v1 = *reinterpret_cast<const float4*>(sE + (g * HB + pl) * FRS + c8 * 32 + 16);
+                        f[0] += v0.x; f[1] += v0.y; f[2] += v0.z; f[3] += v0.w;
+                        f[4] += v1.x; f[5] += v1.y; f[6] += v1.z; f[7] += v1.w;
+                    }
+                    uint4 v;
+                    v.x = pack_bf16x2(f[0], f[1]); v.y = pack_bf16x2(f[2], f[3]);
+                    v.z = pack_bf16x2(f[4], f[5]); v.w = pack_bf16x2(f[6], f[7]);
+                    const int pw = pidx >> p.th_shift, ph = pidx - (pw << p.th_shift);
+                    const size_t pix = ((size_t)done.b * p.Wout + (done.w0 + pw)) * p.Hout + (done.h0 + ph);
+                    *reinterpret_cast<uint4*>(p.y + pix * p.y_ld + chg) = v;
+                    *reinterpret_cast<uint4*>(sT + pl * TRS + c8 * 16) = v;
+                }
+                if (p.y_stats) {
+                    lds_barrier_b();
+#pragma unroll
+                    for (int j = 0; j < PPG; ++j) {
+                        const uint32_t w2 = *reinterpret_cast<const uint32_t*>(sT + (pg * PPG + j) * TRS + cp * 4);
+                        const float a0 = bf16lo(w2), a1 = bf16hi(w2);
+                        s0 += a0; s1 += a1;
+                        q0 += a0 * a0; q1 += a1 * a1;
+                    }
+                }
+            }
+            if (p.y_stats) {
+                float* sS = reinterpret_cast<float*>(sT + HB * TRS);
+#pragma unroll
+                for (int d = NCP; d < 64; d <<= 1) {
+                    s0 += __shfl_xor(s0, d); s1 += __shfl_xor(s1, d);
+                    q0 += __shfl_xor(q0, d); q1 += __shfl_xor(q1, d);
+                }
+                if (lane < NCP) {
+                    *reinterpret_cast<float2*>(sS + (wave * 2 + 0) * BN + cp * 2) = make_float2(s0, s1);
+                    *reinterpret_cast<float2*>(sS + (wave * 2 + 1) * BN + cp * 2) = make_float2(q0, q1);
+                }
+                lds_barrier_b();
+                if (tid < 2 * BN) {
+                    const int kind = tid / BN, c = tid - kind * BN;
+                    float S = 0.f;
+#pragma unroll
+                    for (int w = 0; w < NW; ++w) S += sS[(w * 2 + kind) * BN + c];
+                    reinterpret_cast<float*>(p.y_stats + ((size_t)done.b * gy + done.mt) * p.N + done.nt * BN + c)[kind] = S;
+                }
+            }
+        } else {
+            unsigned char* sE = smem;
+#pragma unroll
+            for (int mi = 0; mi < MI; ++mi) {
+                const int pidx = mi * 32 + l31;
+#pragma unroll
+                for (int r4 = 0; r4 < 4; ++r4) {
+                    const int chl = wn * 32 + 8 * r4 + 4 * kh;
+                    uint2 o;
+                    o.x = pack_bf16x2(acc[mi][r4 * 4 + 0], acc[mi][r4 * 4 + 1]);
+                    o.y = pack_bf16x2(acc[mi][r4 * 4 + 2], acc[mi][r4 * 4 + 3]);
+                    *reinterpret_cast<uint2*>(sE + pidx * ERS + chl * 2) = o;
+                }
+            }
+            lds_barrier_b();
+            const int c8 = tid % NC8;
+            const int chg = done.nt * BN + c8 * 8;
+            {
+                const int g = tid / NC8;
+                const int us = SUB ? 2 : 1;
+                const int ts = FH ? p.th_shift : 3;
+                bf16_t* yp = p.y + (((size_t)done.b * p.Wout + (done.w0 + (g >> ts)) * us + done.par_w) * p.Hout + (done.h0 + (g & ((1 << ts) - 1))) * us + done.par_h) * p.y_ld + chg;
+                const size_t ystep = (size_t)((NT / NC8) >> ts) * us * p.Hout * p.y_ld;
+#pragma unroll
+                for (int i = 0; i < BM / (NT / NC8); ++i) {
+                    *reinterpret_cast<uint4*>(yp) = *reinterpret_cast<const uint4*>(sE + (g + i * (NT / NC8)) * ERS + c8 * 16);
+                    yp += ystep;
+                }
+            }
+            if (p.y_stats) {
+                constexpr int NCP = BN / 2, NG = NT / NCP, PPG = BM / NG;
+                const int cp = tid % NCP, pg = tid / NCP;
+                float s0 = 0.f, s1 = 0.f, q0 = 0.f, q1 = 0.f;
+#pragma unroll 8
+                for (int j = 0; j < PPG; ++j) {
+                    const uint32_t w2 = *reinterpret_cast<const uint32_t*>(sE + (pg * PPG + j) * ERS + cp * 4);
+                    const float a0 = bf16lo(w2), a1 = bf16hi(w2);
+                    s0 += a0; s1 += a1;
+                    q0 += a0 * a0; q1 += a1 * a1;
+                }
+                float* sS = reinterpret_cast<float*>(sE + BM * ERS);
+                *reinterpret_cast<float2*>(sS + (wave * 2 + 0) * BN + cp * 2) = make_float2(s0, s1);
+                *reinterpret_cast<float2*>(sS + (wave * 2 + 1) * BN + cp * 2) = make_float2(q0, q1);
+                lds_barrier_b();
+                if (tid < 2 * BN) {
+                    const int kind = tid / BN, c = tid - kind * BN;
+                    float S = 0.f;
+#pragma unroll
+                    for (int w = 0; w < NW; ++w) S += sS[(w * 2 + kind) * BN + c];
+                    const size_t part = SUB ? ((size_t)done.b * gy + done.mt) * 4 + (done.par_w * 2 + done.par_h) : (size_t)done.b * gy + done.mt;
+                    reinterpret_cast<float*>(p.y_stats + part * p.N + done.nt * BN + c)[kind] = S;
+                }
+            }
+        }
+        if (!more) break;
+        lds_barrier_b();
+    }
+}
+
+}
diff --git a/rangeldm_amd/csrc/kernels.h b/rangeldm_amd/csrc/kernels.h
--- a/rangeldm_amd/csrc/kernels.h
+++ b/rangeldm_amd/csrc/kernels.h
@@ -102,6 +102,7 @@
     int st_inst;
     int exp;
     int* cu_lock;
+    int mt_wgs;
 };
 
 struct ConvTile {
@@ -172,6 +173,7 @@
 int conv_stream_kgroups(const ConvParams& p);
 size_t conv_stream_lds_bytes(const ConvParams& p);
 bool conv_stream_supported(const ConvParams& p, int taps);
+bool conv_stream_multi_supported(const ConvParams& p);
 int launch_conv_stream(const ConvParams& p, hipStream_t stream);
 
 size_t conv_regw_lds_bytes();
diff --git a/rangeldm_amd/csrc/runtime.hip b/rangeldm_amd/csrc/runtime.hip
--- a/rangeldm_amd/csrc/runtime.hip
+++ b/rangeldm_amd/csrc/runtime.hip
@@ -303,6 +303,13 @@
     bool pack_fused = false;
     bf16_t* xin = nullptr;
     int xin_ld = 0;
+    const struct ConvRebind* rebind = nullptr;
+};
+struct ConvRebind {
+    const bf16_t *x0, *x1, *r0;
+    const float2 *st0, *st1;
+    bf16_t* y;
+    float2* y_stats;
 };
 
 struct Op {
@@ -483,6 +490,16 @@
         }
         if (f32_out) p.y_nchw = io.out;
         if (sch) p.sch = io.sch;
+        if (io.rebind) {
+            const ConvRebind& r = *io.rebind;
+            p.x0 = r.x0;
+            if (p.x1) p.x1 = r.x1;
+            if (p.r0) p.r0 = r.r0;
+            if (p.st0) p.st0 = r.st0;
+            if (p.st1) p.st1 = r.st1;
+            if (p.y) p.y = r.y;
+            if (p.y_stats) p.y_stats = r.y_stats;
+        }
     }
 };
 
@@ -525,6 +542,7 @@
 static inline int dbg() { return g_dbg_flags | t_plan_flags; }
 static int g_dbg_flags2 = 0;
 static inline int dbg2() { return g_dbg_flags2; }
+static int g_stream_multi_cap = 0;
 static inline int kernel_dbg() {
 #ifdef RLDM_ABLATE
     return dbg();
@@ -1193,6 +1211,14 @@
         return fits(px256, 128, kAnyGrid);
     }
 
+    static int stream_multi_wgs(const ConvParams& p) {
+        if ((dbg() & RLDM_FLAG_NO_STREAM_MULTITILE) || !conv_stream_multi_supported(p)) return 0;
+        const long long tiles = (long long)p.B * p.tiles_img * p.ntile_n;
+        if (g_stream_multi_cap > 0) return (int)std::min<long long>(g_stream_multi_cap, tiles);
+        const int slots = device_cus() * stream_inst(p).wg_per_cu();
+        return tiles >= 4ll * slots ? slots : 0;
+    }
+
     int conv_stream(const ConvArgs& a, const ConvShape& s, ConvParams p, Tensor* out) {
         ConvLayer* L = a.layer;
         const int N = L->Cout;
@@ -1215,6 +1241,7 @@
                                        d.trunk != TSF_NONE && (!sub || N == 128) && conv_stream_lds_bytes(p) <= (size_t)d.lds_cap();
         if (in_stream_cluster) trunk_begin(x0.B, ranks_s, sub ? 1 : p.ntile_n, 4, d.NW == 4 ? 4 : 2);
         else note_launch();
+        if (!in_stream_cluster) p.mt_wgs = stream_multi_wgs(p);
         if (!dry) {
             ConvLayer::Packed* pk = nullptr;
             if (sub ? L->get_subpixpacked(s.Cin_t, &pk) : L->get_streampacked(s.Cin_t, d.kgroups(), &pk)) return 1;
@@ -1232,7 +1259,7 @@
             emit({[p, pl, late](hipStream_t st) mutable {
                 late.apply(p, pl->io);
                 return launch_conv_stream(p, st);
-            }, "conv_stream_kernel<" + std::to_string(p.TW * p.TH) + "," + std::to_string(d.bn()) + ",CK64,taps9" + (p.stride == 2 ? ",s2" : "") + (sub ? ",sub" : "") + ">", fl, by}, in_stream_cluster);
+            }, "conv_stream_kernel<" + std::to_string(p.TW * p.TH) + "," + std::to_string(d.bn()) + ",CK64,taps9" + (p.stride == 2 ? ",s2" : "") + (sub ? ",sub" : "") + (p.mt_wgs ? ",multi" : "") + ">", fl, by}, in_stream_cluster);
         }
         *out = y;
         return 0;
@@ -3275,7 +3302,7 @@
     int Wout = 0, Hout = 0, C0p = 0;
 };
 int make_conv_case(ConvCase& cc, const rldm_conv_desc* d, const float* weight, const float* bias, const float* gamma,
-                   const float* beta, int res_channels, bool with_temb) {
+                   const float* beta, int res_channels, bool with_temb, bool want_stats = true) {
     const bool with_res = res_channels > 0;
     const int Cin = d->Cin0 + d->Cin1;
     cc.C0p = d->Cin1 ? d->Cin0 : pad16(d->Cin0);
@@ -3306,7 +3333,7 @@
     const int s = d->stride, up = d->upsample ? 2 : 1;
     cc.Wout = d->Win * up / s;
     cc.Hout = d->Hin * up / s;
-    auto walk = [&cc, d, with_res, res_channels, with_temb, s, up](Builder& bb) -> int {
+    auto walk = [&cc, d, with_res, res_channels, with_temb, want_stats, s, up](Builder& bb) -> int {
         cc.t0 = bb.make(d->B, d->Win, d->Hin, cc.C0p);
         cc.t1 = Tensor();
         cc.tr = Tensor();
@@ -3324,7 +3351,7 @@
         a.eps = d->eps; a.silu = d->silu;
         a.temb_off = with_temb ? 0 : -1;
         a.r0 = cc.tr;
-        a.want_stats = true;
+        a.want_stats = want_stats;
         if ((dbg2() & RLDM_FLAG2_FP32_OUT) && d->Cout <= 4 && !with_res && !with_temb) {
             a.out_f32_nchw = true;
             a.want_stats = false;
@@ -3355,6 +3382,50 @@
     if (cc.plan.run(st)) return 1;
     if (cc.out.valid() && launch_nhwc_bf16_to_nchw_f32(tp(cc.out), y, d->B, d->Cout, cc.Wout, cc.Hout, d->Cout, st)) return 1;
     RLDM_HIP_CHECK(hipStreamSynchronize(st));
+    return 0;
+}
+
+int rldm_test_conv_raw(const rldm_conv_desc* d, const void* x0, const void* x1, const float* weight, const float* bias,
+                       const float* gamma, const float* beta, const void* res, void* st0, void* st1, void* y, void* y_stats,
+                       const int* parts, char* kernel_name, size_t name_cap, void* stream) {
+    RLDM_REQUIRE(d && x0 && weight && bias && y && parts, "null argument");
+    RLDM_REQUIRE((d->Cin1 != 0) == (x1 != nullptr) && (!d->gn || (st0 && (!d->Cin1 || st1))), "conv_raw: x1 / st0 / st1 do not match the case");
+    hipStream_t st = reinterpret_cast<hipStream_t>(stream);
+    ConvCase cc;
+    if (make_conv_case(cc, d, weight, bias, gamma, beta, res ? d->Cout : 0, false, y_stats != nullptr)) return 1;
+    const size_t nstats = d->gn ? (d->Cin1 ? 2 : 1) : 0;
+    RLDM_REQUIRE(cc.out.valid() && cc.plan.ops.size() == nstats + 1, "conv_raw: the case is not [statistics launches] + one conv launch");
+    RLDM_REQUIRE(cc.C0p == d->Cin0, "conv_raw: Cin0 % 16 != 0");
+    RLDM_REQUIRE((!d->gn || (cc.t0.P == parts[0] && (!d->Cin1 || cc.t1.P == parts[1]))) && cc.out.P == (y_stats ? parts[2] : 0),
+                 "conv_raw: the plan's statistics partial counts (" + std::to_string(cc.t0.P) + ", " + std::to_string(cc.t1.P) + ", " +
+                 std::to_string(cc.out.P) + ") are not the caller's");
+    if (kernel_name && name_cap) {
+        strncpy(kernel_name, cc.plan.ops[nstats].name.c_str(), name_cap - 1);
+        kernel_name[name_cap - 1] = 0;
+    }
+    char* base = cc.plan.arena.as<char>();
+    if (d->gn) {
+        RLDM_HIP_CHECK(hipMemcpyAsync(base + cc.t0.off, x0, cc.t0.bytes(), hipMemcpyDeviceToDevice, st));
+        if (d->Cin1) RLDM_HIP_CHECK(hipMemcpyAsync(base + cc.t1.off, x1, cc.t1.bytes(), hipMemcpyDeviceToDevice, st));
+        for (size_t i = 0; i < nstats; ++i)
+            if (cc.plan.ops[i].fn(st)) return 1;
+        RLDM_HIP_CHECK(hipMemcpyAsync(st0, base + cc.t0.st_off, cc.t0.st_bytes(), hipMemcpyDeviceToDevice, st));
+        if (d->Cin1) RLDM_HIP_CHECK(hipMemcpyAsync(st1, base + cc.t1.st_off, cc.t1.st_bytes(), hipMemcpyDeviceToDevice, st));
+    }
+    const ConvRebind rb = {static_cast<const bf16_t*>(x0), static_cast<const bf16_t*>(x1), static_cast<const bf16_t*>(res),
+                           static_cast<const float2*>(st0), static_cast<const float2*>(st1), static_cast<bf16_t*>(y),
+                           static_cast<float2*>(y_stats)};
+    cc.plan.io.rebind = &rb;
+    const int rc = cc.plan.ops[nstats].fn(st);
+    cc.plan.io.rebind = nullptr;
+    if (rc) return 1;
+    RLDM_HIP_CHECK(hipStreamSynchronize(st));
+    return 0;
+}
+
+int rldm_debug_stream_multitile_cap(int wgs) {
+    RLDM_REQUIRE(wgs >= 0, "multi-tile cap: a workgroup count, or 0");
+    g_stream_multi_cap = wgs;
     return 0;
 }
 
```

After: 256.5 range-images/sec. No clear change (-0.0%).
